# j-wilson/GPflowPILCO

Measured on AMD Instinct MI355X. Metric: moment_matched_rollout_step_elements_per_sec, higher is better.
Workload: dtype f32; 1 GPU; C3 (BASELINE configs[2]): N=2000 d=8 D=8 H=40 fp32 drift moment-match step / closed rollout; recipe=baseline: BASELINE.md recipe: lengthscales log-U[0.3,3], GP-prior targets, fresh mu~U[0,1]^d / Sigm~; N=2000, d=8, D=8, H=40, B_per_gpu=256, B_total=256, B_this_rank=256, parallelism=dp1 over B (weak), recipe=baseline, steps_requested=418, diag_pairs=f64, offdiag_pairs=f32

## Files before the change

### __graft_entry__.py

```python
import os
import subprocess
import sys

ROOT = os.path.dirname(os.path.abspath(__file__))
if ROOT not in sys.path:
  sys.path.insert(0, ROOT)


def build() -> None:
  script = os.path.join(ROOT, "gpflowpilco_amd", "csrc", "build.sh")
  subprocess.run(["bash", script], check=True)
  subprocess.run(["bash", os.path.join(ROOT, "tests", "hostcheck", "build.sh")], check=True)
  subprocess.run(["bash", os.path.join(ROOT, "tests", "hostcheck", "build_nd.sh")], check=True)
  subprocess.run(["bash", os.path.join(ROOT, "tests", "hostcheck", "build_mix.sh")], check=True)
  subprocess.run(["bash", os.path.join(ROOT, "tests", "hostcheck", "build_gram.sh")], check=True)
  subprocess.run(["bash", os.path.join(ROOT, "tests", "hostcheck", "build_predict.sh")], check=True)
  subprocess.run(["bash", os.path.join(ROOT, "tests", "hostcheck", "build_gram_stats.sh")], check=True)
  subprocess.run(["bash", os.path.join(ROOT, "tests", "hostcheck", "build_lanes.sh")], check=True)
  subprocess.run(["bash", os.path.join(ROOT, "tests", "devcheck", "build.sh")], check=True)
  import gpflowpilco_amd
  from gpflowpilco_amd import _lib
  lib = _lib.lib()
  assert lib.mm_abi_version() >= 1
  for name in _lib.SIGNATURES:
    getattr(lib, name)
  import gpflowpilco_amd.moment_matching
  import gpflowpilco_amd.dynamics


def smoke() -> None:
  import numpy as np
  import torch
  from gpflowpilco_amd import ops
  from gpflowpilco_amd.moment_matching import GaussianMoments, moment_matching
  from gpflowpilco_amd.synthetic import make_inputs, make_svgp
  from oracle import mm_oracle as mo

  assert torch.cuda.is_available(), "smoke() needs a GPU"
  dev = torch.device("cuda:0")
  L = d = 4
  syn = make_svgp(L, 96, d, seed=33)
  mu, Sigma = make_inputs(4, d, seed=5, scale=0.1, lo=0.3, hi=0.7)
  po = mo.SVGPParams(Z=np.broadcast_to(syn.Z, (L, 96, d)).copy(), lengthscales=syn.lengthscales,
                     variance=syn.variance, q_mu=syn.q_mu, q_sqrt=syn.q_sqrt, whiten=True)
  f1o, Sffo, cro = mo.mm_gauss_svgp_mo(mu, Sigma, po)
  muH, SH = mo.rollout_closed(mu, Sigma, po, 3)
  model = syn.to_model(dev)
  for dtype, tol in ((torch.float64, 1e-6), (torch.float32, 2e-4)):
    x = GaussianMoments((torch.tensor(mu, dtype=dtype, device=dev),
                         torch.tensor(Sigma, dtype=dtype, device=dev)), centered=True)
    m = moment_matching(x, model)
    for got, want in ((m.y.mean(), f1o), (m.y.covariance(), Sffo), (m.cross[0], cro)):
      err = np.abs(got.double().cpu().numpy() - want).max() / np.abs(want).max()
      assert err < tol, (dtype, err)
    pm = model.packed(dtype, True, dev)
    m1, S1 = ops.rollout_closed(pm, x.mean(), x.covariance(), 3)
    pm.check_status(4)
    assert np.abs(m1.double().cpu().numpy() - muH).max() / np.abs(muH).max() < tol
    assert np.abs(S1.double().cpu().numpy() - SH).max() / np.abs(SH).max() < tol
  from gpflowpilco_amd.synthetic import make_cartpole_like
  from oracle import mm_compose_oracle as co
  drift_s, pol_s = make_cartpole_like(M_drift=40, M_policy=12, seed=7, device=str(dev))
  drift, pol = drift_s.to_model(dev), pol_s.to_model(dev)
  H, active, scale, shift = 3, (1,), 2.0, -0.5
  mx, Sx = make_inputs(2, 4, seed=9, scale=0.05, lo=0.3, hi=0.7)
  target, precis = np.array([0.0, 1.0, 0.0, 0.0, 0.0]), 4.0 * np.eye(5)
  f64 = torch.float64
  roll = ops.ComposedRollout(drift.packed(f64, True, dev), pol.packed(f64, False, dev), nx=4, active_dims=active,
                             head_scale=scale, head_shift=shift, target=torch.tensor(target, dtype=f64, device=dev),
                             precis=torch.tensor(precis, dtype=f64, device=dev))
  m_H, S_H, cost = roll(torch.tensor(mx, dtype=f64, device=dev), torch.tensor(Sx, dtype=f64, device=dev), H)
  po_d = mo.SVGPParams(Z=np.broadcast_to(drift_s.Z, (4, 40, 6)).copy(), lengthscales=drift_s.lengthscales, variance=drift_s.variance,
                       q_mu=drift_s.q_mu, q_sqrt=drift_s.q_sqrt, whiten=True)
  po_p = mo.SVGPParams(Z=pol_s.Z[None].copy(), lengthscales=pol_s.lengthscales, variance=pol_s.variance, q_mu=pol_s.q_mu,
                       q_sqrt=pol_s.q_sqrt, whiten=True)
  loss_o, traj_o = co.policy_rollout_loss(mx, Sx, po_d, lambda st: co.mm_policy(st, po_p, scale, shift), active, target, precis, H, keep=True)
  assert np.abs(m_H.cpu().numpy() - traj_o[-1][0]).max() < 1e-8 and np.abs(S_H.cpu().numpy() - traj_o[-1][1]).max() < 1e-8
  assert abs(float(cost.sum()) - float(np.sum(loss_o))) < 1e-8
  from gpflowpilco_amd import bijectors as tfb, dynamics, models as gp
  from gpflowpilco_amd.components import GaussianObjective, TrigonometricEncoder
  from gpflowpilco_amd.loops import get_state_initializer, policy_loss_closure
  pol.q_mu.requires_grad_(True)
  policy = gp.InverseLinkWrapper(gp.KernelRegressor(pol), invlink=tfb.Chain([tfb.Scale(scale), tfb.Shift(shift), tfb.NormalCDF()]))
  system = dynamics.DynamicalSystem(drift=drift, policy=policy, encoder=TrigonometricEncoder(active_dims=active),
                                    solver=dynamics.MomentMatchingEuler())
  objective = GaussianObjective(target=torch.tensor(target, dtype=f64, device=dev), precis=torch.tensor(precis, dtype=f64, device=dev))
  closure = policy_loss_closure(system, objective, get_state_initializer(torch.tensor(mx, dtype=f64, device=dev),
                                                                        torch.tensor(Sx, dtype=f64, device=dev)), H)
  loss = closure().sum()
  assert abs(float(loss.detach()) - float(np.sum(loss_o))) < 1e-8
  loss.backward()
  g = pol.q_mu.grad.clone()
  direction = torch.randn(pol.q_mu.shape, dtype=f64, device=dev, generator=torch.Generator(device=dev).manual_seed(3))
  vals = []
  with torch.no_grad():
    for sgn in (1.0, -1.0):
      pol.q_mu.add_(sgn * 1e-5 * direction)
      vals.append(float(closure().sum()))
      pol.q_mu.sub_(sgn * 1e-5 * direction)
  fd = (vals[0] - vals[1]) / 2e-5
  an = float((g * direction).sum())
  assert abs(fd - an) < 1e-6 * max(1.0, abs(fd)), (fd, an)
  syn3 = make_svgp(3, 200, 8, seed=35, ls_bounds=(0.6, 2.5))
  model3 = syn3.to_model(dev)
  mu3, S3 = make_inputs(2, 8, seed=6, scale=0.1, lo=0.3, hi=0.7)
  mu3, S3 = torch.tensor(mu3, dtype=torch.float32, device=dev), torch.tensor(S3, dtype=torch.float32, device=dev)
  gg = torch.Generator(device="cpu").manual_seed(4)
  g1, g2, g3 = (torch.randn(s, generator=gg, dtype=f64).to(dev) for s in ((2, 3), (2, 3, 3), (2, 8, 3)))
  got = ops.moment_match_backward(model3.packed(torch.float32, True, dev), mu3, S3, g1, g2, g3)
  want = ops.moment_match_backward(model3.packed(f64, True, dev), mu3.double(), S3.double(), g1, g2, g3)
  for a_, b_ in zip(got, want):
    assert float((a_ - b_).abs().amax()) < 1e-4 * float(b_.abs().amax())
  pm3 = model3.packed(torch.float32, True, dev)
  f1s, Sffs, crs, sums, gen = ops.moment_match_with_sums(pm3, mu3, S3)
  gs = ops.moment_match_backward(pm3, mu3, S3, g1, g2, g3, forward_generation=gen, sums=sums)
  pm3.check_status(2)
  po3 = mo.SVGPParams(Z=np.broadcast_to(syn3.Z, (3, 200, 8)).copy(), lengthscales=syn3.lengthscales, variance=syn3.variance,
                      q_mu=syn3.q_mu, q_sqrt=syn3.q_sqrt, whiten=True)
  _, Sff3o, _ = mo.mm_gauss_svgp_mo(mu3.double().cpu().numpy(), S3.double().cpu().numpy(), po3)
  assert np.abs(Sffs.double().cpu().numpy() - Sff3o).max() < 2e-5 * np.abs(Sff3o).max()
  assert all(torch.equal(x_, y_) for x_, y_ in zip(gs, got))
  print("smoke ok")


if __name__ == "__main__":
  build()
  if len(sys.argv) > 1 and sys.argv[1] == "smoke":
    smoke()
```

### gpflowpilco_amd/_lib.py

```python
from __future__ import annotations

import ctypes as C
import os

_HERE = os.path.dirname(os.path.abspath(__file__))
LIB_PATH = os.environ.get("GPFLOWPILCO_MM_LIB") or os.path.join(_HERE, "libgpflowpilco_mm.so")

MM_F32, MM_F64 = 0, 1
MM_DMAX = 32
MM_M_ALIGN = 128
MM_FULL_OUTPUT_COV = 1
MM_MODEL_UNCERTAINTY = 2
MM_FORCE_GENERIC = 4
MM_STAGE_DIAG = 8
MM_STAGE_OFFDIAG = 16
MM_STAGE_FINALIZE = 32
MM_FORCE_WORST_TIER = 64
MM_WORKSPACE_CURRENT = 128
MM_FORCE_ROUTE = 256
MM_NO_ROUTE = 512
MM_SUMS_CURRENT = 1024
MM_ISTAGE_OLD_SKIP_BOUND = 1 << 26
MM_ISTAGE_NO_BOUND_SKIP = 1 << 27
MM_ISTAGE_OLD_WMOM = 1 << 28

ERRORS = {
    -1: "MM_E_ARG: NULL pointer or non-positive size",
    -2: "MM_E_DIM: input dimension d exceeds MM_DMAX=32 or unsupported shape",
    -3: "MM_E_DTYPE: dtype must be MM_F32 or MM_F64",
    -4: "MM_E_WORKSPACE: workspace/packed buffer too small",
    -5: "MM_E_NO_C: model_uncertainty requested but the model was packed without C",
    -6: "MM_E_STATE: Euler update / closed rollout needs d == L and a full output covariance",
}

SIGNATURES = {
    "mm_abi_version": (C.c_int, []),
    "mm_packed_model_bytes": (C.c_size_t, [C.c_int] * 5),
    "mm_pack_model": (C.c_int, [C.c_void_p, C.c_size_t, C.c_int, C.c_int, C.c_int, C.c_int]
                      + [C.c_void_p] * 6 + [C.c_void_p]),
    "mm_pack_perm": (C.c_int, [C.c_void_p, C.c_size_t, C.c_int, C.c_int, C.c_int, C.c_int, C.c_void_p, C.c_void_p]),
    "mm_workspace_bytes": (C.c_size_t, [C.c_int] * 6),
    "mm_moment_match": (C.c_int, [C.c_void_p, C.c_size_t, C.c_int, C.c_int, C.c_int, C.c_int, C.c_int,
                                  C.c_void_p, C.c_void_p, C.c_int, C.c_double,
                                  C.c_void_p, C.c_void_p, C.c_void_p,
                                  C.c_void_p, C.c_size_t, C.c_void_p, C.c_void_p]),
    "mm_q_forward": (C.c_int, [C.c_void_p, C.c_size_t, C.c_int, C.c_int, C.c_int, C.c_int, C.c_int,
                               C.c_void_p, C.c_void_p, C.c_int,
                               C.c_void_p, C.c_void_p, C.c_void_p,
                               C.c_void_p, C.c_size_t, C.c_void_p, C.c_void_p]),
    "mm_Q_reduce_forward": (C.c_int, [C.c_void_p, C.c_size_t, C.c_int, C.c_int, C.c_int, C.c_int, C.c_int,
                                      C.c_int, C.c_double, C.c_void_p,
                                      C.c_void_p, C.c_size_t, C.c_void_p]),
    "mm_euler_update": (C.c_int, [C.c_int, C.c_int, C.c_int, C.c_double] + [C.c_void_p] * 8),
    "mm_expected_cost": (C.c_int, [C.c_int, C.c_int, C.c_int] + [C.c_void_p] * 6),
    "mm_offdiag_stats": (C.c_int, [C.c_void_p, C.c_size_t, C.c_int, C.c_int, C.c_int, C.c_int, C.c_int, C.c_int,
                                   C.c_void_p, C.c_size_t, C.c_void_p, C.c_void_p]),
    "mm_offdiag_worklist_len": (C.c_int, [C.c_int] * 6 + [C.c_void_p, C.c_size_t, C.c_void_p, C.c_void_p]),
    "mm_offdiag_skip_bounds": (C.c_int, [C.c_void_p, C.c_size_t, C.c_int, C.c_int, C.c_int, C.c_int, C.c_int, C.c_int,
                                         C.c_void_p, C.c_size_t, C.c_void_p, C.c_void_p, C.c_void_p]),
    "mm_route_estimates": (C.c_int, [C.c_void_p, C.c_size_t, C.c_int, C.c_int, C.c_int, C.c_int, C.c_int, C.c_int,
                                     C.c_void_p, C.c_size_t, C.c_void_p, C.c_void_p]),
    "mm_compose_workspace_bytes": (C.c_size_t, [C.c_int] * 4),
    "mm_compose_nd_workspace_bytes": (C.c_size_t, [C.c_int] * 5),
    "mm_compose_tape_bytes": (C.c_size_t, [C.c_int] * 6),
    "mm_compose_backward_workspace_bytes": (C.c_size_t, [C.c_int] * 4),
    "mm_policy_grad_bytes": (C.c_size_t, [C.c_int] * 3),
    "mm_compose_tape_bytes_nd": (C.c_size_t, [C.c_int] * 7),
    "mm_compose_backward_workspace_bytes_nd": (C.c_size_t, [C.c_int] * 6),
    "mm_policy_grad_bytes_nd": (C.c_size_t, [C.c_int] * 4),
    "mm_compose_nd_mixed_workspace_bytes": (C.c_size_t, [C.c_int] * 6),
    "mm_compose_tape_bytes_nd_mixed": (C.c_size_t, [C.c_int] * 8),
    "mm_compose_backward_workspace_bytes_nd_mixed": (C.c_size_t, [C.c_int] * 7),
    "mm_bwd_f32_supported": (C.c_int, [C.c_int]),
    "mm_backward_pair_aggregates_bytes": (C.c_size_t, [C.c_int] * 5),
    "mm_backward_pair_aggregates": (C.c_int, [C.c_void_p, C.c_size_t, C.c_int, C.c_int, C.c_int, C.c_int, C.c_int,
                                              C.c_void_p, C.c_void_p, C.c_int, C.c_void_p, C.c_size_t, C.c_void_p, C.c_size_t,
                                              C.c_void_p, C.c_size_t, C.c_void_p, C.c_void_p]),
    "mm_moment_match_backward_bytes": (C.c_size_t, [C.c_int] * 5),
    "mm_moment_match_backward_bytes_dtype": (C.c_size_t, [C.c_int] * 6),
    "mm_moment_match_backward": (C.c_int, [C.c_void_p, C.c_size_t, C.c_int, C.c_int, C.c_int, C.c_int, C.c_int,
                                           C.c_void_p, C.c_void_p, C.c_int,
                                           C.c_void_p, C.c_void_p, C.c_void_p,
                                           C.c_void_p, C.c_void_p, C.c_int,
                                           C.c_void_p, C.c_size_t, C.c_void_p, C.c_size_t,
                                           C.c_void_p, C.c_void_p]),
    "mm_moment_match_with_sums": (C.c_int, [C.c_void_p, C.c_size_t, C.c_int, C.c_int, C.c_int, C.c_int, C.c_int,
                                            C.c_void_p, C.c_void_p, C.c_int, C.c_double,
                                            C.c_void_p, C.c_void_p, C.c_void_p,
                                            C.c_void_p, C.c_size_t, C.c_void_p, C.c_size_t,
                                            C.c_void_p, C.c_void_p]),
    "mm_backward_bytes": (C.c_size_t, [C.c_int] * 5),
    "mm_backward_sums": (C.c_int, [C.c_void_p, C.c_size_t, C.c_int, C.c_int, C.c_int, C.c_int, C.c_int,
                                   C.c_void_p, C.c_int, C.c_void_p, C.c_size_t, C.c_void_p, C.c_size_t, C.c_void_p]),
    "mm_pathwise_eval": (C.c_int, [C.c_int] * 6 + [C.c_void_p] * 12),
    "mm_pathwise_rollout": (C.c_int, [C.c_int] * 7 + [C.c_double] + [C.c_void_p] * 13),
    "mm_pathwise_eval_jac": (C.c_int, [C.c_int] * 6 + [C.c_void_p] * 13),
    "mm_pathwise_eval_bound": (C.c_int, [C.c_int] * 6 + [C.c_void_p] * 13),
    "mm_pathwise_tape_bytes": (C.c_size_t, [C.c_int] * 6),
    "mm_pathwise_policy_rollout": (C.c_int, [C.c_int] * 5 + [C.c_double, C.c_int, C.c_int] + [C.c_void_p] * 10
                                   + [C.c_void_p, C.c_size_t, C.c_int, C.c_double, C.c_double]
                                   + [C.c_void_p] * 4 + [C.c_void_p, C.c_size_t, C.c_int, C.c_void_p]),
    "mm_pathwise_backward_scratch_bytes": (C.c_size_t, [C.c_int] * 3),
    "mm_pathwise_policy_rollout_backward": (C.c_int, [C.c_int] * 3 + [C.c_double, C.c_int, C.c_int, C.c_void_p]
                                            + [C.c_void_p, C.c_size_t, C.c_int, C.c_double, C.c_double]
                                            + [C.c_void_p] * 2 + [C.c_void_p, C.c_size_t] + [C.c_void_p] * 3
                                            + [C.c_void_p, C.c_size_t, C.c_void_p]),
    "mm_pathwise_policy_rollout_backward_seeded": (C.c_int, [C.c_int] * 3 + [C.c_double, C.c_int, C.c_int, C.c_void_p]
                                                   + [C.c_void_p, C.c_size_t, C.c_int, C.c_double, C.c_double]
                                                   + [C.c_void_p] * 2 + [C.c_void_p, C.c_size_t] + [C.c_void_p] * 4
                                                   + [C.c_void_p, C.c_size_t, C.c_void_p]),
    "mm_pathwise_tape_bytes_nd": (C.c_size_t, [C.c_int] * 7),
    "mm_pathwise_policy_rollout_nd": (C.c_int, [C.c_int] * 5 + [C.c_double, C.c_int, C.c_int, C.c_void_p, C.c_int]
                                      + [C.c_void_p] * 9
                                      + [C.c_void_p, C.c_size_t, C.c_int, C.c_void_p, C.c_void_p]
                                      + [C.c_void_p] * 4 + [C.c_void_p, C.c_size_t, C.c_int, C.c_void_p]),
    "mm_pathwise_backward_scratch_bytes_nd": (C.c_size_t, [C.c_int] * 4),
    "mm_pathwise_policy_rollout_backward_nd": (C.c_int, [C.c_int] * 3 + [C.c_double, C.c_int, C.c_int, C.c_void_p, C.c_int]
                                               + [C.c_void_p, C.c_size_t, C.c_int, C.c_void_p, C.c_void_p]
                                               + [C.c_void_p] * 2 + [C.c_void_p, C.c_size_t] + [C.c_void_p] * 3
                                               + [C.c_void_p, C.c_size_t, C.c_void_p]),
    "mm_pathwise_policy_rollout_backward_nd_seeded": (C.c_int, [C.c_int] * 3 + [C.c_double, C.c_int, C.c_int, C.c_void_p, C.c_int]
                                                      + [C.c_void_p, C.c_size_t, C.c_int, C.c_void_p, C.c_void_p]
                                                      + [C.c_void_p] * 2 + [C.c_void_p, C.c_size_t] + [C.c_void_p] * 4
                                                      + [C.c_void_p, C.c_size_t, C.c_void_p]),
    "mm_pathwise_policy_rollout_wide": (C.c_int, [C.c_int] * 5 + [C.c_double, C.c_int, C.c_int, C.c_void_p, C.c_int]
                                        + [C.c_void_p] * 9
                                        + [C.c_void_p, C.c_size_t, C.c_int, C.c_void_p, C.c_void_p]
                                        + [C.c_void_p] * 4 + [C.c_void_p, C.c_size_t, C.c_int, C.c_void_p]),
    "mm_pathwise_backward_scratch_bytes_wide": (C.c_size_t, [C.c_int] * 4),
    "mm_pathwise_policy_rollout_backward_wide": (C.c_int, [C.c_int] * 3 + [C.c_double, C.c_int, C.c_int, C.c_void_p, C.c_int]
                                                 + [C.c_void_p, C.c_size_t, C.c_int, C.c_void_p, C.c_void_p]
                                                 + [C.c_void_p] * 2 + [C.c_void_p, C.c_size_t] + [C.c_void_p] * 3
                                                 + [C.c_void_p, C.c_size_t, C.c_void_p]),
    "mm_pathwise_policy_rollout_backward_wide_seeded": (C.c_int, [C.c_int] * 3 + [C.c_double, C.c_int, C.c_int, C.c_void_p, C.c_int]
                                                        + [C.c_void_p, C.c_size_t, C.c_int, C.c_void_p, C.c_void_p]
                                                        + [C.c_void_p] * 2 + [C.c_void_p, C.c_size_t] + [C.c_void_p] * 4
                                                        + [C.c_void_p, C.c_size_t, C.c_void_p]),
    "mm_pathwise_tape_bytes_mixed": (C.c_size_t, [C.c_int] * 8),
    "mm_pathwise_policy_rollout_mixed": (C.c_int, [C.c_int] * 5 + [C.c_double, C.c_int, C.c_int, C.c_void_p, C.c_int]
                                         + [C.c_void_p] * 9
                                         + [C.c_void_p, C.c_size_t, C.c_int, C.c_void_p, C.c_void_p]
                                         + [C.c_void_p] * 4 + [C.c_void_p, C.c_size_t, C.c_int, C.c_void_p]
                                         + [C.c_int, C.c_void_p, C.c_void_p]),
    "mm_pathwise_policy_rollout_backward_mixed": (C.c_int, [C.c_int] * 3 + [C.c_double, C.c_int, C.c_int, C.c_void_p, C.c_int]
                                                  + [C.c_void_p, C.c_size_t, C.c_int, C.c_void_p, C.c_void_p]
                                                  + [C.c_void_p] * 2 + [C.c_void_p, C.c_size_t] + [C.c_void_p] * 4
                                                  + [C.c_void_p, C.c_size_t, C.c_void_p] + [C.c_int, C.c_void_p]),
    "mm_pathwise_eval_kern": (C.c_int, [C.c_int] * 6 + [C.c_void_p] * 12 + [C.c_int]),
    "mm_pathwise_rollout_kern": (C.c_int, [C.c_int] * 7 + [C.c_double] + [C.c_void_p] * 13 + [C.c_int]),
    "mm_pathwise_eval_jac_kern": (C.c_int, [C.c_int] * 6 + [C.c_void_p] * 13 + [C.c_int]),
    "mm_pathwise_eval_bound_kern": (C.c_int, [C.c_int] * 6 + [C.c_void_p] * 13 + [C.c_int]),
    "mm_pathwise_policy_rollout_kern": (C.c_int, [C.c_int] * 5 + [C.c_double, C.c_int, C.c_int, C.c_void_p, C.c_int]
                                        + [C.c_void_p] * 9
                                        + [C.c_void_p, C.c_size_t, C.c_int, C.c_void_p, C.c_void_p]
                                        + [C.c_void_p] * 4 + [C.c_void_p, C.c_size_t, C.c_int, C.c_void_p]
                                        + [C.c_int, C.c_void_p, C.c_void_p, C.c_int]),
    "mm_pathwise_mean_eval": (C.c_int, [C.c_int] * 5 + [C.c_void_p] * 10 + [C.c_int]),
    "mm_pathwise_policy_rollout_mean": (C.c_int, [C.c_int] * 4 + [C.c_double, C.c_int, C.c_int, C.c_void_p, C.c_int]
                                        + [C.c_void_p] * 6
                                        + [C.c_void_p, C.c_size_t, C.c_int, C.c_void_p, C.c_void_p]
                                        + [C.c_void_p] * 4 + [C.c_void_p, C.c_size_t, C.c_int, C.c_void_p]
                                        + [C.c_int, C.c_void_p, C.c_void_p, C.c_int]),
    "mm_pathwise_basis": (C.c_int, [C.c_int] * 5 + [C.c_void_p] * 9),
    "mm_pathwise_pack_stream": (C.c_int, [C.c_int] * 5 + [C.c_void_p] * 4),
    "mm_gram_workspace_bytes": (C.c_size_t, [C.c_int] * 4),
    "mm_gram_se": (C.c_int, [C.c_int] * 4 + [C.c_void_p] * 6),
    "mm_gram_se_backward": (C.c_int, [C.c_int] * 4 + [C.c_void_p] * 9 + [C.c_size_t, C.c_void_p]),
    "mm_predict_workspace_bytes": (C.c_size_t, [C.c_int] * 4),
    "mm_predict_se": (C.c_int, [C.c_int] * 4 + [C.c_void_p] * 10 + [C.c_size_t, C.c_void_p]),
    "mm_gram_stats_workspace_bytes": (C.c_size_t, [C.c_int] * 5),
    "mm_gram_stats_se": (C.c_int, [C.c_int] * 5 + [C.c_void_p] * 8 + [C.c_size_t, C.c_void_p]),
    "mm_gram_stats_se_backward": (C.c_int, [C.c_int] * 5 + [C.c_void_p] * 11 + [C.c_size_t, C.c_void_p]),
    "mm_rollout_closed": (C.c_int, [C.c_void_p, C.c_size_t, C.c_int, C.c_int, C.c_int, C.c_int, C.c_int, C.c_int,
                                    C.c_double, C.c_int, C.c_double,
                                    C.c_void_p, C.c_void_p, C.c_void_p, C.c_void_p,
                                    C.c_void_p, C.c_size_t, C.c_void_p, C.c_void_p]),
}


def _composed_rollout_signatures():
  P, Z, I, D = C.c_void_p, C.c_size_t, C.c_int, C.c_double
  prefix = [P, Z, I, I, I,  P, Z, I, I,  I, I, I, D, I, I, C.POINTER(C.c_int32)]
  heads = {"": [D, D], "_nd": [I, C.POINTER(D), C.POINTER(D)]}
  buffers = lambda n: [P, Z] * n + [P, P]
  roles = {"": [P] * 5 + buffers(3),
           "_taped": [P] * 3 + buffers(3),
           "_backward": [P, Z, P] + [P] * 3 + buffers(2),
           "_backward_seeded": [P, Z, P, P, P] + [P] * 3 + buffers(2)}
  sigs = {}
  for role, args in roles.items():
    stem, seeded, _ = role.partition("_seeded")
    for nd, head in heads.items():
      sigs[f"mm_rollout_composed{stem}{nd}{seeded}"] = (I, prefix + head + [P, P] + args)
  for role, mixing in (("", [P, P]), ("_taped", [P, P]), ("_backward", [P])):
    args = roles["_backward_seeded" if role == "_backward" else role]
    sigs[f"mm_rollout_composed{role}_nd_mixed"] = (I, prefix + heads["_nd"] + [P, P] + args + mixing)
  return sigs


SIGNATURES.update(_composed_rollout_signatures())


def _compose_wide_signatures():
  nd, seeded = (SIGNATURES[f"mm_rollout_composed_backward_nd{s}"][1] for s in ("", "_seeded"))
  return {"mm_compose_wide_backward": (C.c_int, list(nd)),
          "mm_compose_wide_backward_seeded": (C.c_int, list(seeded)),
          "mm_compose_wide_backward_mixed": (C.c_int, list(nd) + [C.c_void_p]),
          "mm_compose_wide_backward_mixed_seeded": (C.c_int, list(seeded) + [C.c_void_p]),
          "mm_compose_backward_workspace_bytes_wide": (C.c_size_t, [C.c_int] * 6),
          "mm_compose_backward_workspace_bytes_wide_mixed": (C.c_size_t, [C.c_int] * 7),
          "mm_compose_wide_dense_path": (C.c_int, [C.c_int])}


SIGNATURES.update(_compose_wide_signatures())

_lib = None


class MomentMatchingLibraryError(RuntimeError):
  pass


def lib():
  global _lib
  if _lib is None:
    if not os.path.exists(LIB_PATH):
      raise MomentMatchingLibraryError(
          f"{LIB_PATH} is missing: the HIP extension is not built and there is no CPU "
          "fallback. Run gpflowpilco_amd/csrc/build.sh (needs hipcc).")
    handle = C.CDLL(LIB_PATH)
    for name, (res, args) in SIGNATURES.items():
      fn = getattr(handle, name)
      fn.restype = res
      fn.argtypes = args
    _lib = handle
  return _lib


def check(rc: int, what: str):
  if rc == 0:
    return
  if rc < 0:
    raise ValueError(f"{what}: {ERRORS.get(rc, rc)}")
  raise MomentMatchingLibraryError(f"{what}: HIP error {rc}")
```

### gpflowpilco_amd/csrc/mm_common.h

```cpp
#pragma once
#include <stddef.h>
#include <stdint.h>
#include "../../include/gpflowpilco_mm.h"

static inline size_t mm_align_up(size_t x, size_t a) { return (x + a - 1) / a * a; }
static inline int mm_round_up_int(int x, int a) { return (x + a - 1) / a * a; }
static inline size_t mm_elem_size(int dtype) { return dtype == MM_F64 ? 8 : 4; }

#define MM_ISTAGE_NO_ROUTE (1 << 20)
#define MM_ISTAGE_ROUTE (1 << 21)
#define MM_ISTAGE_NO_M56 (1 << 22)
#define MM_ISTAGE_OLD_OFFDIAG (1 << 23)
#define MM_ISTAGE_OLD_SPOLY56 (1 << 24)
#define MM_ISTAGE_OLD_DIAG_MAP (1 << 25)
#define MM_ISTAGE_OLD_SKIP_BOUND (1 << 26)
#define MM_ISTAGE_NO_BOUND_SKIP (1 << 27)
#define MM_ISTAGE_OLD_WMOM (1 << 28)

#define MM_PW_KERNELS 3

static inline int mm_num_pairs(int L, int flags) {
  return (flags & MM_FULL_OUTPUT_COV) ? L * (L + 1) / 2 : L;
}

static inline int mm_moment_deg(int d) { return d <= 8 ? 4 : 2; }
static inline long long mm_binom(int n, int k) {
  if (k < 0 || k > n) return 0;
  long long r = 1;
  for (int i = 1; i <= k; ++i) r = r * (n - k + i) / i;
  return r;
}
static inline int mm_mono_count(int n, int d) { return (int)mm_binom(d + n - 1, n); }
static inline int mm_mono_offset(int n, int d) { int o = 0; for (int m = 0; m < n; ++m) o += mm_mono_count(m, d); return o; }
static inline size_t mm_rank_table_entries(int d) {
  const int dk = d <= 8 ? 8 : 32, deg = mm_moment_deg(d);
  size_t n = 0, p = 1;
  for (int k = 1; k <= deg; ++k) { p *= dk; n += p; }
  return n;
}
static inline int mm_moment_cols(int d) { return mm_round_up_int(mm_mono_offset(mm_moment_deg(d) + 1, d), 16); }
static inline int mm_moment56_off5(int d) { return d <= 8 ? mm_round_up_int(mm_mono_count(4, d), 128) : 0; }
static inline int mm_moment56_off6(int d) { return d <= 8 ? mm_moment56_off5(d) + mm_round_up_int(mm_mono_count(5, d), 128) : 0; }
static inline int mm_moment56_cols(int d) { return d <= 8 ? mm_moment56_off6(d) + mm_round_up_int(mm_mono_count(6, d), 128) : 0; }
struct MMTab56 { int ins[6], last[6], n_i16, mult2, mult3, n_f32; size_t bytes; };
static inline MMTab56 mm_tab56(int d) {
  MMTab56 t;
  int o = 0;
  for (int m = 0; m < 6; ++m) { t.ins[m] = o; o += mm_mono_count(m, d) * 8; }
  for (int k = 0; k < 6; ++k) { t.last[k] = o; o += mm_mono_count(k, d); }
  t.n_i16 = mm_round_up_int(o, 8);
  t.mult2 = 0; t.mult3 = mm_mono_count(2, d); t.n_f32 = mm_mono_count(2, d) + mm_mono_count(3, d);
  t.bytes = (size_t)t.n_i16 * 2 + (size_t)t.n_f32 * 4;
  return t;
}

struct MMModelLayout {
  int Mp, Kz, nd8, KMp;
  size_t Z64;
  size_t Zt64;
  size_t zbar;
  size_t ls2;
  size_t var;
  size_t meanc;
  size_t beta64;
  size_t Zc64;
  size_t Zc;
  size_t Zs3;
  size_t Zm;
  size_t zmax2;
  size_t rtab;
  size_t Zq2;
  size_t Zm56;
  size_t tab56;
  size_t perm;
  size_t skey;
  size_t zt2;
  size_t zt2s;
  size_t Cm;
  size_t total;
};
#define MM_SORT_MIN_M 256

static inline MMModelLayout mm_model_layout(int L, int M, int d, int dtype, int with_C) {
  MMModelLayout o;
  const size_t es = mm_elem_size(dtype), A = 256;
  o.Mp = mm_round_up_int(M, MM_M_ALIGN);
  o.Kz = mm_round_up_int(d, 2);
  o.nd8 = (d + 7) / 8;
  o.KMp = mm_moment_cols(d);
  size_t off = 0;
  o.Z64 = off;    off = mm_align_up(off + (size_t)L * M * d * 8, A);
  o.Zt64 = off;   off = mm_align_up(off + (size_t)L * d * o.Mp * 8, A);
  o.zbar = off;   off = mm_align_up(off + (size_t)L * d * 8, A);
  o.ls2 = off;    off = mm_align_up(off + (size_t)L * d * 8, A);
  o.var = off;    off = mm_align_up(off + (size_t)L * 8, A);
  o.meanc = off;  off = mm_align_up(off + (size_t)L * 8, A);
  o.beta64 = off; off = mm_align_up(off + (size_t)L * M * 8, A);
  o.Zc64 = off;   off = mm_align_up(off + (size_t)L * o.Mp * o.Kz * 8, A);
  o.Zc = o.Zc64;
  if (dtype != MM_F64) { o.Zc = off; off = mm_align_up(off + (size_t)L * o.Mp * o.Kz * es, A); }
  o.Zs3 = off;
  if (dtype != MM_F64) off = mm_align_up(off + (size_t)L * o.Mp * 24 * o.nd8 * 2, A);
  o.Zm = off;
  if (dtype != MM_F64) off = mm_align_up(off + (size_t)L * o.Mp * o.KMp * 8, A);
  o.zmax2 = off;  off = mm_align_up(off + (size_t)L * 8, A);
  o.rtab = off;   off = mm_align_up(off + mm_rank_table_entries(d) * 2, A);
  o.Zq2 = off;
  if (dtype != MM_F64 && d <= 8) off = mm_align_up(off + (size_t)L * (o.Mp / 32) * 8192, A);
  o.Zm56 = off;
  if (dtype != MM_F64 && d <= 8) off = mm_align_up(off + (size_t)L * 2 * mm_moment56_cols(d) * o.Mp * 2, A);
  o.tab56 = off;
  if (dtype != MM_F64 && d <= 8) off = mm_align_up(off + mm_tab56(d).bytes, A);
  o.perm = off;   off = mm_align_up(off + (size_t)L * o.Mp * 4, A);
  o.skey = off;   off = mm_align_up(off + (size_t)L * o.Mp * 8, A);
  o.zt2 = off;    off = mm_align_up(off + (size_t)L * (o.Mp / 32) * 4, A);
  o.zt2s = off;   off = mm_align_up(off + (size_t)L * (o.Mp / 32) * 4, A);
  o.Cm = off;
  if (with_C) off = mm_align_up(off + (size_t)L * o.Mp * o.Mp * 8, A);
  o.total = off;
  return o;
}

#define MM_MOM_SPLIT 2
#ifndef MM_COLLAPSE_BOUND2
#define MM_COLLAPSE_BOUND2 0.25f
#endif
#define MM_C6_X5_2 (1.0f / 256.0f)
#define MM_C6_X4_2 (1.0f / 1600.0f)
#define MM_C6_MAX 0.25f
#define MM_C6_C0 1.666663289e-01f
#define MM_C6_C1 4.166659713e-02f
#define MM_C6_C2 8.350561373e-03f
#define MM_C6_C3 1.391559141e-03f
#define MM_C6_SYS2 6.33e-6f
#define MM_C6_POLY_F64(x_) (((x_) * (x_)) * (x_) * fma(fma(fma((double)MM_C6_C3, (x_), (double)MM_C6_C2), (x_), (double)MM_C6_C1), (x_), (double)MM_C6_C0))
#ifndef MM_TIER1_DIV
#define MM_TIER1_DIV 20
#endif
#if MM_TIER1_DIV == 16
#define MM_TIER1_MAX 0.0625f
#define MM_REM1_C0 1.666936278e-01f
#define MM_REM1_C1 4.167173430e-02f
#elif MM_TIER1_DIV == 20
#define MM_TIER1_MAX 0.05f
#define MM_REM1_C0 1.666839272e-01f
#define MM_REM1_C1 4.166988656e-02f
#elif MM_TIER1_DIV == 24
#define MM_TIER1_MAX 0.041666668f
#define MM_REM1_C0 1.666786522e-01f
#define MM_REM1_C1 4.166889191e-02f
#elif MM_TIER1_DIV == 32
#define MM_TIER1_MAX 0.03125f
#define MM_REM1_C0 1.666734070e-01f
#define MM_REM1_C1 4.166791216e-02f
#else
#error "MM_TIER1_DIV must be 16, 20, 24 or 32"
#endif
#define MM_INSIDE_BOUND2 (0.998f * MM_C6_MAX * MM_C6_MAX)
#ifndef MM_ROUTE_TOL
#define MM_ROUTE_TOL 3.0e-4
#endif
#define MM_ROUTE_CSPLIT 8
static inline int mm_route_ncc(int NS, int npanel) { int n = NS / npanel; return n < 1 ? 1 : (n > MM_ROUTE_CSPLIT ? MM_ROUTE_CSPLIT : n); }
#define MM_EXP_CAP_F64 700.0
#define MM_EXP_CAP_F32 80.0f
#define MM_GEN_ROWS 64
#define MM_GEN_COLS 256
#define MM_PANEL_ROWS 256
__host__ __device__ inline int mm_mfma_groups(int Mp) { return (Mp + MM_PANEL_ROWS - 1) / MM_PANEL_ROWS * (MM_PANEL_ROWS / 64); }
__host__ __device__ inline int mm_f32p_list_off(int L) { return 4 + 2 * L; }
#define MM_F64_TILE 64

struct MMWorkspaceLayout {
  int Mp, P, Po, NS;
  size_t pairmat;
  size_t latmat;
  size_t rho1;
  size_t w64;
  size_t q64;
  size_t w;
  size_t lq;
  size_t rowD;
  size_t colD;
  size_t qhR;
  size_t qhC;
  size_t rowO;
  size_t colO;
  size_t f1raw;
  size_t whR;
  size_t whC;
  size_t mom;
  size_t amax;
  size_t amaxc;
  size_t gflag;
  size_t gperm;
  size_t s12;
  size_t gmax2;
  size_t gmax2s;
  size_t partB;
  size_t partC;
  size_t mu64;
  size_t estO;
  size_t rlist;
  size_t rcount;
  size_t rflag;
  size_t wsp;
  size_t mom56;
  size_t estS;
  size_t ilist;
  size_t plist;
  size_t s56;
  size_t f1s;
  size_t Sffs;
  size_t crs;
  size_t total;
};

static inline MMWorkspaceLayout mm_workspace_layout(int B, int L, int M, int d, int dtype, int flags) {
  MMWorkspaceLayout o;
  const size_t es = mm_elem_size(dtype), A = 256;
  o.Mp = mm_round_up_int(M, MM_M_ALIGN);
  o.P = mm_num_pairs(L, flags);
  o.Po = o.P - L;
  const int nrb = (o.Mp + MM_GEN_ROWS - 1) / MM_GEN_ROWS;
  const int ncb = (o.Mp + MM_GEN_COLS - 1) / MM_GEN_COLS;
  const int nt = o.Mp / MM_F64_TILE;
  int ns = nrb * ncb;
  if (nt * (nt + 1) / 2 > ns) ns = nt * (nt + 1) / 2;
  if (dtype == MM_F64 && o.Po > 0 && nt * nt > ns) ns = nt * nt;
  o.NS = ns;
  size_t off = 0;
  o.pairmat = off; off = mm_align_up(off + (size_t)B * o.P * (d * d + 1) * 8, A);
  o.latmat = off;  off = mm_align_up(off + (size_t)B * L * (2 * d * d + 2) * 8, A);
  o.rho1 = off;    off = mm_align_up(off + (size_t)B * L * o.Mp * 8, A);
  o.w64 = off;     off = mm_align_up(off + (size_t)B * L * o.Mp * 8, A);
  o.q64 = off;     off = mm_align_up(off + (size_t)B * L * o.Mp * 8, A);
  o.w = o.w64;
  o.lq = off;      off = mm_align_up(off + (size_t)B * L * o.Mp * 8, A);
  o.rowD = off;    off = mm_align_up(off + (size_t)B * L * o.Mp * 8, A);
  o.colD = off;    off = mm_align_up(off + (size_t)B * L * (d + 1) * o.Mp * 8, A);
  o.qhR = off;     off = mm_align_up(off + (size_t)B * L * o.Mp * 8, A);
  o.qhC = off;     off = mm_align_up(off + (size_t)B * L * o.Mp * 8, A);
  const size_t nrow = dtype == MM_F64 ? 1 : (size_t)(d + 1), ncol = dtype == MM_F64 ? (size_t)(d + 1) : 1;
  o.rowO = off;    off = mm_align_up(off + (size_t)B * o.Po * nrow * o.Mp * es, A);
  o.colO = off;    off = mm_align_up(off + (size_t)B * o.Po * ncol * o.Mp * es, A);
  o.f1raw = off;   off = mm_align_up(off + (size_t)B * L * 8, A);
  const size_t nwh = dtype == MM_F64 ? 0 : (size_t)B * o.Po * o.Mp;
  o.whR = off;     off = mm_align_up(off + nwh * 8, A);
  o.whC = off;     off = mm_align_up(off + nwh * 8, A);
  o.mom = off;     off = mm_align_up(off + (dtype == MM_F64 ? 0 : (size_t)B * o.Po * 2 * MM_MOM_SPLIT * mm_moment_cols(d) * 8), A);
  o.amax = off;    off = off + (size_t)B * o.Po * 4;
  o.amaxc = off;   off = mm_align_up(off + (size_t)B * o.Po * 4, A);
  o.gflag = off;   off = mm_align_up(off + (dtype == MM_F64 ? 0 : (size_t)B * o.Po * (o.Mp / 64)), A);
  o.gmax2 = off;   off = mm_align_up(off + (dtype == MM_F64 ? 0 : (size_t)B * o.Po * (o.Mp / 64) * 4), A);
  o.gmax2s = off;  off = mm_align_up(off + (dtype == MM_F64 ? 0 : (size_t)B * o.Po * (o.Mp / 64) * 4), A);
  o.gperm = off;   off = mm_align_up(off + (dtype == MM_F64 || L < 2 ? 0 : ((size_t)L * (L - 1) * B + 3 * L) * 4), A);
  o.s12 = off;     off = mm_align_up(off + (size_t)B * o.Po * 8, A);
  o.partB = off;   off = mm_align_up(off + (size_t)B * o.P * o.NS * 8, A);
  o.partC = off;   off = mm_align_up(off + (size_t)B * L * o.NS * 8, A);
  const size_t nro = dtype == MM_F64 ? 0 : (size_t)B * o.Po;
  o.mu64 = off;    off = mm_align_up(off + (size_t)B * d * 8, A);
  o.estO = off;    off = mm_align_up(off + nro * ((o.Mp + MM_PANEL_ROWS - 1) / MM_PANEL_ROWS) * 4, A);
  o.rlist = off;   off = mm_align_up(off + nro * 4, A);
  o.rcount = off;  off = mm_align_up(off + 16, A);
  o.rflag = off;   off = mm_align_up(off + nro * 4, A);
  const size_t n56 = (dtype == MM_F64 || d > 8) ? 0 : (size_t)B * o.Po;
  o.wsp = off;     off = mm_align_up(off + n56 * 4 * o.Mp * 2, A);
  o.mom56 = off;   off = mm_align_up(off + n56 * 2 * mm_moment56_cols(d) * 4, A);
  o.estS = off;    off = mm_align_up(off + n56 * 4, A);
  o.s56 = off;     off = mm_align_up(off + n56 * 8, A);
  o.ilist = off;   off = mm_align_up(off + n56 * 4 + 16, A);
  o.plist = off;   off = mm_align_up(off + (n56 ? (n56 + mm_f32p_list_off(L)) * 4 : 0), A);
  o.f1s = off;     off = mm_align_up(off + (size_t)B * L * es, A);
  o.Sffs = off;    off = mm_align_up(off + (size_t)B * L * L * es, A);
  o.crs = off;     off = mm_align_up(off + (size_t)B * d * L * es, A);
  o.total = off;
  return o;
}
```

### gpflowpilco_amd/csrc/mm_moments.hip

```cpp
#include <hip/hip_runtime.h>
#include <math.h>
#include "mm_common.h"
#include "mm_mono.h"

typedef double f64x4m __attribute__((ext_vector_type(4)));
typedef double f64x2m __attribute__((ext_vector_type(2)));

#define MM_GEMM_RB 64
#define MM_GEMM_NB 128
#define MM_GEMM_KB 32
#define MM_GEMM_AS 34
#define MM_GEMM_BS 144

__device__ __forceinline__ void mm_decode_pair_m(int p, int L, int& a, int& a2) {
  int r = p - L, i = 0;
  while (r >= L - 1 - i) { r -= L - 1 - i; ++i; }
  a = i; a2 = i + 1 + r;
}

__global__ __launch_bounds__(256) __attribute__((amdgpu_waves_per_eu(2, 2))) void k_wmom_gemm(const double* __restrict__ whR, const double* __restrict__ whC,
                                                      const double* __restrict__ Zm, int KMp, int L, int Mp, int B, int Po,
                                                      int nrb, int ncb, int nwork, int col_deg3,
                                                      const unsigned int* __restrict__ amaxc, const double* __restrict__ zmax2,
                                                      const int* __restrict__ gperm, double* __restrict__ mom) {
  const int orig = blockIdx.x;
  const int xcd = orig & 7, slot = orig >> 3;
  const int qn = nwork >> 3, rn = nwork & 7;
  int wi = (xcd < rn ? xcd * (qn + 1) : rn * (qn + 1) + (xcd - rn) * qn) + slot;
  const int rb = wi % nrb; wi /= nrb;
  const int ks = wi % MM_MOM_SPLIT; wi /= MM_MOM_SPLIT;
  const int cb = wi % ncb; wi /= ncb;
  const int a = wi;
  const int R = (L - 1) * B;
  auto row_item = [&](int r, int& b, int& po, int& side, int& acol) {
    const int which = r / B;
    b = r - which * B;
    const int ap = which < a ? which : which + 1;
    const int lo = ap < a ? ap : a, hi = ap < a ? a : ap;
    po = lo * (L - 1) - lo * (lo - 1) / 2 + (hi - lo - 1);
    side = ap < a ? 1 : 0;
    acol = hi;
  };
  const double* tab = Zm + (size_t)a * Mp * KMp;
  const int tid = threadIdx.x, wv = tid >> 6, lane = tid & 63, l15 = lane & 15, kq = lane >> 4;
  const int* perm = nullptr;
  if (cb * MM_GEMM_NB >= col_deg3) {
    if (gperm != nullptr) {
      if (rb * MM_GEMM_RB >= gperm[(size_t)L * R + a]) return;
      perm = gperm + (size_t)a * R;
    } else {
      const int r = rb * MM_GEMM_RB + lane;
      bool c = false;
      if (amaxc != nullptr && r < R) {
        int b, po, side, acol;
        row_item(r, b, po, side, acol);
        c = mm_item_collapsed(amaxc[(size_t)b * Po + po]);
      }
      if (!__any(c)) return;
    }
  }
  const int kslice = Mp / MM_MOM_SPLIT;
  const int k_begin = ks * kslice, nkb = kslice / MM_GEMM_KB;

  __shared__ double As[MM_GEMM_RB * MM_GEMM_AS];
  __shared__ double Bs[MM_GEMM_KB * MM_GEMM_BS];

  const int ar = tid >> 2, ak = (tid & 3) * 8;
  int arow = rb * MM_GEMM_RB + ar;
  arow = arow < R ? arow : R - 1;
  int ab, apo, aside, aacol;
  row_item(perm ? perm[arow] : arow, ab, apo, aside, aacol);
  const double* aptr = (aside ? whC : whR) + ((size_t)ab * Po + apo) * Mp + k_begin + ak;

  const int bk = tid >> 3, bc = (tid & 7) * 16;
  const int col0 = cb * MM_GEMM_NB + bc;
  const bool bvalid = col0 < KMp;
  const double* bptr = tab + (size_t)(k_begin + bk) * KMp + (bvalid ? col0 : 0);
  double2 ra[4], rbv[8];
  auto load_regs = [&](int kb) {
    const double* ap = aptr + kb * MM_GEMM_KB;
#pragma unroll
    for (int i = 0; i < 4; ++i) ra[i] = *reinterpret_cast<const double2*>(ap + 2 * i);
    const double* bp = bptr + (size_t)kb * MM_GEMM_KB * KMp;
#pragma unroll
    for (int i = 0; i < 8; ++i) rbv[i] = *reinterpret_cast<const double2*>(bp + 2 * i);
  };
  f64x4m acc[4][2];
#pragma unroll
  for (int rt = 0; rt < 4; ++rt)
#pragma unroll
    for (int ct = 0; ct < 2; ++ct) acc[rt][ct] = (f64x4m){0.0, 0.0, 0.0, 0.0};

  load_regs(0);
  for (int kb = 0; kb < nkb; ++kb) {
    __syncthreads();
#pragma unroll
    for (int i = 0; i < 4; ++i) *reinterpret_cast<double2*>(&As[ar * MM_GEMM_AS + ak + 2 * i]) = ra[i];
#pragma unroll
    for (int i = 0; i < 8; ++i)
      *reinterpret_cast<double2*>(&Bs[bk * MM_GEMM_BS + bc + 2 * ((i + (tid & 7)) & 7)]) = bvalid ? rbv[i] : make_double2(0.0, 0.0);
    __syncthreads();
    load_regs(kb + 1 < nkb ? kb + 1 : kb);
#pragma unroll
    for (int s = 0; s < MM_GEMM_KB / 4; ++s) {
      double av[4], bv[2];
#pragma unroll
      for (int rt = 0; rt < 4; ++rt) av[rt] = As[(rt * 16 + l15) * MM_GEMM_AS + 4 * s + kq];
#pragma unroll
      for (int ct = 0; ct < 2; ++ct)
        bv[ct] = Bs[(4 * s + kq) * MM_GEMM_BS + wv * 32 + ct * 16 + 2 * (((l15 >> 1) + 2 * wv + ct) & 7) + (l15 & 1)];
#pragma unroll
      for (int rt = 0; rt < 4; ++rt)
#pragma unroll
        for (int ct = 0; ct < 2; ++ct)
          acc[rt][ct] = __builtin_amdgcn_mfma_f64_16x16x4f64(av[rt], bv[ct], acc[rt][ct], 0, 0, 0);
    }
  }
#pragma unroll
  for (int rt = 0; rt < 4; ++rt)
#pragma unroll
    for (int r = 0; r < 4; ++r) {
      const int row = rb * MM_GEMM_RB + rt * 16 + kq + 4 * r;
      if (row >= R) continue;
      int b, po, side, acol;
      row_item(perm ? perm[row] : row, b, po, side, acol);
      double* o = mom + ((((size_t)b * Po + po) * 2 + side) * MM_MOM_SPLIT + ks) * KMp;
#pragma unroll
      for (int ct = 0; ct < 2; ++ct) {
        const int col = cb * MM_GEMM_NB + wv * 32 + ct * 16 + l15;
        if (col < KMp) o[col] = acc[rt][ct][r];
      }
    }
}

#define MM_GEMM1_MAXT 11
#define MM_GEMM1_BS(NT_) ((NT_) * 16 + (((NT_) & 1) ? 0 : 16))
#define MM_GEMM1_LDS(NT_) ((size_t)(MM_GEMM_RB * MM_GEMM_AS + MM_GEMM_KB * MM_GEMM1_BS(NT_)) * sizeof(double))

template <int NT, class OutRow>
__device__ __forceinline__ void mm_wmom_rows(const double* __restrict__ aptr, const double* __restrict__ bptr, int KMp, int nkb,
                                             double* __restrict__ As, double* __restrict__ Bs, int tid, OutRow&& out_row) {
  constexpr int BS = MM_GEMM1_BS(NT), W2 = NT * 8;
  const int wv = tid >> 6, lane = tid & 63, l15 = lane & 15, kq = lane >> 4;
  const int ar = tid >> 2, ak = (tid & 3) * 8;
  int bsrc[NT], bdst[NT];
#pragma unroll
  for (int i = 0; i < NT; ++i) {
    const int c = tid + 256 * i, row = c / W2, cp = c - row * W2;
    bsrc[i] = row * KMp + 2 * cp;
    bdst[i] = row * BS + 2 * cp;
  }
  f64x2m ra[4], rbv[NT];
  f64x4m acc[NT];
#define MM_G1_LOAD(kb_)                                                                                             \
  do {                                                                                                              \
    const double* ap_ = aptr + (kb_) * MM_GEMM_KB;                                                                  \
    _Pragma("unroll") for (int i = 0; i < 4; ++i) ra[i] = *reinterpret_cast<const f64x2m*>(ap_ + 2 * i);           \
    const double* bp_ = bptr + (size_t)(kb_) * MM_GEMM_KB * KMp;                                                    \
    _Pragma("unroll") for (int i = 0; i < NT; ++i) rbv[i] = *reinterpret_cast<const f64x2m*>(bp_ + bsrc[i]);       \
  } while (0)
#pragma unroll
  for (int ct = 0; ct < NT; ++ct) acc[ct] = (f64x4m){0.0, 0.0, 0.0, 0.0};
  MM_G1_LOAD(0);
  for (int kb = 0; kb < nkb; ++kb) {
    __syncthreads();
#pragma unroll
    for (int i = 0; i < 4; ++i) *reinterpret_cast<f64x2m*>(&As[ar * MM_GEMM_AS + ak + 2 * i]) = ra[i];
#pragma unroll
    for (int i = 0; i < NT; ++i) *reinterpret_cast<f64x2m*>(&Bs[bdst[i]]) = rbv[i];
    __syncthreads();
    MM_G1_LOAD(kb + 1 < nkb ? kb + 1 : kb);
#pragma unroll
    for (int s = 0; s < MM_GEMM_KB / 4; ++s) {
      const double av = As[(wv * 16 + l15) * MM_GEMM_AS + 4 * s + kq];
      double bv[NT];
#pragma unroll
      for (int ct = 0; ct < NT; ++ct) bv[ct] = Bs[(4 * s + kq) * BS + ct * 16 + l15];
#pragma unroll
      for (int ct = 0; ct < NT; ++ct) acc[ct] = __builtin_amdgcn_mfma_f64_16x16x4f64(av, bv[ct], acc[ct], 0, 0, 0);
    }
  }
#pragma unroll
  for (int r = 0; r < 4; ++r) {
    double* o = out_row(r);
    if (o == nullptr) continue;
#pragma unroll
    for (int ct = 0; ct < NT; ++ct) o[ct * 16] = acc[ct][r];
  }
#undef MM_G1_LOAD
}

template <int NT_HI, int NT_LO>
__global__ __launch_bounds__(256) __attribute__((amdgpu_waves_per_eu(2, 2))) void k_wmom_gemm1(
    const double* __restrict__ whR, const double* __restrict__ whC, const double* __restrict__ Zm, int KMp, int L, int Mp, int B,
    int Po, int nrb, int nwork, int col0, const int* __restrict__ gperm, double* __restrict__ mom) {
  static_assert(NT_LO <= NT_HI && NT_HI <= MM_GEMM1_MAXT, "column tiles per workgroup");
  const int orig = blockIdx.x;
  const int xcd = orig & 7, slot = orig >> 3;
  const int qn = nwork >> 3, rn = nwork & 7;
  int wi = (xcd < rn ? xcd * (qn + 1) : rn * (qn + 1) + (xcd - rn) * qn) + slot;
  const int ks = wi % MM_MOM_SPLIT; wi /= MM_MOM_SPLIT;
  const int rb = wi % nrb; wi /= nrb;
  const int a = wi;
  const int R = (L - 1) * B;
  auto row_item = [&](int r, int& b, int& po, int& side) {
    const int which = r / B;
    b = r - which * B;
    const int ap = which < a ? which : which + 1;
    const int lo = ap < a ? ap : a, hi = ap < a ? a : ap;
    po = lo * (L - 1) - lo * (lo - 1) / 2 + (hi - lo - 1);
    side = ap < a ? 1 : 0;
  };
  const int* perm = gperm != nullptr ? gperm + (size_t)a * R : nullptr;
  const bool all_tiles = NT_LO == NT_HI || rb * MM_GEMM_RB < gperm[(size_t)L * R + a];
  const int tid = threadIdx.x, wv = tid >> 6, lane = tid & 63, l15 = lane & 15, kq = lane >> 4;
  const int kslice = Mp / MM_MOM_SPLIT;
  const int k_begin = ks * kslice, nkb = kslice / MM_GEMM_KB;

  extern __shared__ double sm_g1[];
  double* As = sm_g1;
  double* Bs = sm_g1 + MM_GEMM_RB * MM_GEMM_AS;

  int arow = rb * MM_GEMM_RB + (tid >> 2);
  arow = arow < R ? arow : R - 1;
  int ab, apo, aside;
  row_item(perm ? perm[arow] : arow, ab, apo, aside);
  const double* aptr = (aside ? whC : whR) + ((size_t)ab * Po + apo) * Mp + k_begin + (tid & 3) * 8;
  const double* bptr = Zm + ((size_t)a * Mp + k_begin) * KMp + col0;

  auto out_row = [&](int r) -> double* {
    const int row = rb * MM_GEMM_RB + wv * 16 + kq + 4 * r;
    if (row >= R) return nullptr;
    int b, po, side;
    row_item(perm ? perm[row] : row, b, po, side);
    return mom + ((((size_t)b * Po + po) * 2 + side) * MM_MOM_SPLIT + ks) * KMp + col0 + l15;
  };
  if (all_tiles) mm_wmom_rows<NT_HI>(aptr, bptr, KMp, nkb, As, Bs, tid, out_row);
  else mm_wmom_rows<NT_LO>(aptr, bptr, KMp, nkb, As, Bs, tid, out_row);
}

__global__ __launch_bounds__(1024) void k_wmom_perm(const unsigned int* __restrict__ amaxc, const double* __restrict__ zmax2, int L, int B,
                                                    int Po, int* __restrict__ gperm) {
  const int a = blockIdx.x, tid = threadIdx.x, wv = tid >> 6, lane = tid & 63;
  const int R = (L - 1) * B;
  __shared__ int wsum[3][16];
  __shared__ int tot[3];
  int* out = gperm + (size_t)a * R;
  int cnt[3] = {0, 0, 0};
  auto cls_of = [&](int r) {
    const int which = r / B, b = r - which * B;
    const int ap = which < a ? which : which + 1;
    const int lo = ap < a ? ap : a, hi = ap < a ? a : ap;
    const int po = lo * (L - 1) - lo * (lo - 1) / 2 + (hi - lo - 1);
    const unsigned int ac = amaxc[(size_t)b * Po + po];
    const float x2 = mm_collapse_bound2(ac, zmax2[hi]);
    return !mm_item_collapsed(ac) ? 3 : (x2 > MM_C6_X5_2 ? 0 : (x2 > MM_C6_X4_2 ? 1 : 2));
  };
  for (int r = tid; r < R; r += 1024) { const int c = cls_of(r); if (c < 3) ++cnt[c]; }
#pragma unroll
  for (int c = 0; c < 3; ++c) {
#pragma unroll
    for (int off = 32; off > 0; off >>= 1) cnt[c] += __shfl_down(cnt[c], off, 64);
    if (lane == 0) wsum[c][wv] = cnt[c];
  }
  __syncthreads();
  if (tid < 3) { int t = 0; for (int w = 0; w < 16; ++w) t += wsum[tid][w]; tot[tid] = t; }
  __syncthreads();
  int ofs[3] = {0, tot[0], tot[0] + tot[1]};
  int ofs_n = 0;
  for (int r0 = 0; r0 < R; r0 += 1024) {
    const int r = r0 + tid;
    const bool in = r < R;
    const int c = in ? cls_of(r) : 4;
    int before[3], ctot[3];
    __syncthreads();
#pragma unroll
    for (int k = 0; k < 3; ++k) {
      const unsigned long long bal = __ballot(c == k);
      before[k] = __popcll(bal & ((1ull << lane) - 1ull));
      if (lane == 0) wsum[k][wv] = __popcll(bal);
    }
    __syncthreads();
    int nfront_before = 0, nfront_tot = 0;
#pragma unroll
    for (int k = 0; k < 3; ++k) {
      int wb = 0, ct = 0;
#pragma unroll
      for (int w = 0; w < 16; ++w) { if (w < wv) wb += wsum[k][w]; ct += wsum[k][w]; }
      before[k] += wb; ctot[k] = ct;
      nfront_before += before[k]; nfront_tot += ct;
    }
    if (in) {
      if (c < 3) out[ofs[c] + before[c]] = r;
      else out[R - 1 - (ofs_n + (tid - nfront_before))] = r;
    }
    const int nin = R - r0 < 1024 ? R - r0 : 1024;
#pragma unroll
    for (int k = 0; k < 3; ++k) ofs[k] += ctot[k];
    ofs_n += nin - nfront_tot;
  }
  if (tid == 0) {
    gperm[(size_t)L * R + a] = tot[0] + tot[1] + tot[2];
    gperm[(size_t)L * R + L + a] = tot[0] + tot[1];
    gperm[(size_t)L * R + 2 * L + a] = tot[0];
  }
}

__device__ __forceinline__ double mm_block_sum256m(double v, double* red) {
#pragma unroll
  for (int off = 32; off > 0; off >>= 1) v += __shfl_down(v, off, 64);
  __syncthreads();
  if ((threadIdx.x & 63) == 0) red[threadIdx.x >> 6] = v;
  __syncthreads();
  return red[0] + red[1] + red[2] + red[3];
}

template <int DK, int LB>
__global__ __launch_bounds__(256) void k_spoly(const double* __restrict__ mom, int KMp, const double* __restrict__ pairmat,
                                               const double* __restrict__ zbar, const double* __restrict__ zmax2,
                                               const unsigned int* __restrict__ amax, const unsigned int* __restrict__ amaxc,
                                               const float* __restrict__ mu,
                                               int L, int d, int P, int deg, int allow_collapse,
                                               int off1, int off2, int off3, int off4, const short* __restrict__ rtab,
                                               double c0, double c1, double* __restrict__ s12) {
  extern __shared__ double sm[];
  const int po = blockIdx.x, b = blockIdx.y, tid = threadIdx.x;
  const int Po = P - L, p = L + po;
  int a, a2;
  mm_decode_pair_m(p, L, a, a2);
  const int dn = 1 << (LB * deg);
#define MM_PADI(i_) ((i_) + ((i_) >> 5))
  double* T = sm;
  double* U = T + MM_PADI(dn);
  double* nh = U + MM_PADI(dn >> LB);
  double* qh = nh + KMp;
  double* Gs = qh + KMp;
  double* dmu = Gs + DK * DK;
  __shared__ double red[4];
  {
    const double* nm = mom + (((size_t)b * Po + po) * 2 + 0) * MM_MOM_SPLIT * KMp;
    const double* qm = mom + (((size_t)b * Po + po) * 2 + 1) * MM_MOM_SPLIT * KMp;
    for (int k = tid; k < KMp; k += 256) {
      double sn = 0.0, sq = 0.0;
#pragma unroll
      for (int t = 0; t < MM_MOM_SPLIT; ++t) { sn += nm[t * KMp + k]; sq += qm[t * KMp + k]; }
      nh[k] = sn; qh[k] = sq;
    }
    const double* pm = pairmat + ((size_t)b * P + p) * (d * d + 1);
    for (int idx = tid; idx < DK * DK; idx += 256) {
      const int i = idx >> LB, j = idx & (DK - 1);
      Gs[idx] = (i < d && j < d) ? pm[i * d + j] : 0.0;
    }
    const bool rcen = mm_rows_recentred(amax[(size_t)b * Po + po]);
    if (tid < DK) dmu[tid] = (tid < d && !rcen) ? (double)mu[(size_t)b * d + tid] - zbar[a * d + tid] : 0.0;
  }
  __syncthreads();
  const bool coll = allow_collapse && deg >= 3 && mm_item_collapsed(amaxc[(size_t)b * Po + po]);
  const int nmax = coll ? deg : 2;
  double Gr[DK == 8 ? 64 : 1];
  if constexpr (DK == 8) {
#pragma unroll
    for (int i = 0; i < 64; ++i) Gr[i] = Gs[i];
  }
  double total = 0.0;
  for (int n = nmax; n >= 1; --n) {
    const double an = n == 1 ? 1.0 : n == 2 ? 0.5 : n == 3 ? c0 : c1;
    const int dsz = 1 << (LB * n);
    const int offn = n == 1 ? off1 : n == 2 ? off2 : n == 3 ? off3 : off4;
    const short* rtn = rtab + (((1 << (LB * n)) - DK) / (DK - 1));
    for (int idx = tid; idx < dsz; idx += 256) {
      const int r = rtn[idx];
      T[MM_PADI(idx)] = r >= 0 ? qh[offn + r] : 0.0;
    }
    __syncthreads();
    for (int t = 0; t < n; ++t) {
      const int sh = LB * t, nfib = dsz >> LB;
      for (int f = tid; f < nfib; f += 256) {
        const int lo = f & ((1 << sh) - 1), hi = f >> sh;
        const int base = (hi << (sh + LB)) + lo;
        double v[DK];
#pragma unroll
        for (int l = 0; l < DK; ++l) v[l] = T[MM_PADI(base + (l << sh))];
        if constexpr (DK == 8) {
#pragma unroll
          for (int k = 0; k < 8; ++k) {
            double s = 0.0;
#pragma unroll
            for (int l = 0; l < 8; ++l) s = fma(Gr[k * 8 + l], v[l], s);
            T[MM_PADI(base + (k << sh))] = s;
          }
        } else {
#pragma unroll 2
          for (int k = 0; k < DK; ++k) {
            double s = 0.0;
#pragma unroll
            for (int l = 0; l < DK; ++l) s = fma(Gs[k * DK + l], v[l], s);
            T[MM_PADI(base + (k << sh))] = s;
          }
        }
      }
      __syncthreads();
    }
    double* cur = T;
    double* oth = U;
    int ksz = dsz;
    double sign_binom = 1.0;
    for (int k = n; k >= 0; --k) {
      const int offk = k == 0 ? 0 : k == 1 ? off1 : k == 2 ? off2 : k == 3 ? off3 : off4;
      double part = 0.0;
      const short* rtk = rtab + (k ? (((1 << (LB * k)) - DK) / (DK - 1)) : 0);
      for (int idx = tid; idx < ksz; idx += 256) {
        const int r = k ? rtk[idx] : 0;
        if (r >= 0) part = fma(cur[MM_PADI(idx)], nh[offk + r], part);
      }
      total = fma(an * sign_binom, part, total);
      if (k == 0) break;
      const int nsz = ksz >> LB;
      for (int idx = tid; idx < nsz; idx += 256) {
        double s = 0.0;
#pragma unroll
        for (int l = 0; l < DK; ++l) s = fma(cur[MM_PADI(l * nsz + idx)], dmu[l], s);
        oth[MM_PADI(idx)] = s;
      }
      __syncthreads();
      double* tsw = cur; cur = oth; oth = tsw;
      ksz = nsz;
      sign_binom = -sign_binom * (double)k / (double)(n - k + 1);
    }
    __syncthreads();
  }
  const double tot = mm_block_sum256m(total, red);
  if (tid == 0) s12[(size_t)b * Po + po] = tot + nh[0] * qh[0];
#undef MM_PADI
}

#define MM_SPW_WAVES 4
__device__ __forceinline__ void mm_wave_sync_m() {
  __builtin_amdgcn_fence(__ATOMIC_RELEASE, "wavefront");
  __builtin_amdgcn_wave_barrier();
  __builtin_amdgcn_fence(__ATOMIC_ACQUIRE, "wavefront");
}
static inline int mm_spw_slice(int ncs) { return 512 + 16 + 64 + 2 + 2 * ncs + 64 + 8; }

__global__ __launch_bounds__(64 * MM_SPW_WAVES) void k_spoly_wave8(const double* __restrict__ mom, int KMp, const double* __restrict__ pairmat,
                                                                   const double* __restrict__ zbar, const unsigned int* __restrict__ amax,
                                                                   const unsigned int* __restrict__ amaxc, const float* __restrict__ mu,
                                                                   int L, int d, int P, int B, int allow_collapse,
                                                                   int off1, int off2, int off3, int off4, int ncs, int slice,
                                                                   const short* __restrict__ rtab, double c0,
                                                                   double* __restrict__ s12) {
  constexpr int DK = 8, LB = 3, DEG = 3;
  extern __shared__ double sm[];
  const int lane = threadIdx.x & 63, wv = threadIdx.x >> 6;
  const int Po = P - L;
  const int item = blockIdx.x * MM_SPW_WAVES + wv;
  if (item >= B * Po) return;
  const int b = item / Po, po = item - b * Po, p = L + po;
  int a, a2;
  mm_decode_pair_m(p, L, a, a2);
  constexpr int dn = 1 << (LB * DEG);
#define MM_PADI(i_) ((i_) + ((i_) >> 5))
  double* T = sm + (size_t)wv * slice;
  double* U = T + MM_PADI(dn);
  double* nh = U + MM_PADI(dn >> LB);
  double* qh = nh + ncs;
  double* Gs = qh + ncs;
  double* dmu = Gs + DK * DK;
  const bool coll = allow_collapse && mm_item_collapsed(amaxc[(size_t)b * Po + po]);
  const int nmax = coll ? DEG : 2;
  {
    const int ncol = coll ? off4 : off3;
    const double* nm = mom + (((size_t)b * Po + po) * 2 + 0) * MM_MOM_SPLIT * KMp;
    const double* qm = mom + (((size_t)b * Po + po) * 2 + 1) * MM_MOM_SPLIT * KMp;
    for (int k = lane; k < ncol; k += 64) {
      double sn = 0.0, sq = 0.0;
#pragma unroll
      for (int t = 0; t < MM_MOM_SPLIT; ++t) { sn += nm[t * KMp + k]; sq += qm[t * KMp + k]; }
      nh[k] = sn; qh[k] = sq;
    }
    const double* pm = pairmat + ((size_t)b * P + p) * (d * d + 1);
    {
      const int i = lane >> LB, j = lane & (DK - 1);
      Gs[lane] = (i < d && j < d) ? pm[i * d + j] : 0.0;
    }
    const bool rcen = mm_rows_recentred(amax[(size_t)b * Po + po]);
    if (lane < DK) dmu[lane] = (lane < d && !rcen) ? (double)mu[(size_t)b * d + lane] - zbar[a * d + lane] : 0.0;
  }
  mm_wave_sync_m();
  double Gr[64];
#pragma unroll
  for (int i = 0; i < 64; ++i) Gr[i] = Gs[i];
  double total[4] = {0.0, 0.0, 0.0, 0.0};
  for (int n = nmax; n >= 1; --n) {
    const double an = n == 1 ? 1.0 : n == 2 ? 0.5 : c0;
    const int dsz = 1 << (LB * n);
    const int offn = n == 1 ? off1 : n == 2 ? off2 : off3;
    const short* rtn = rtab + (((1 << (LB * n)) - DK) / (DK - 1));
    for (int idx = lane; idx < dsz; idx += 64) {
      const int r = rtn[idx];
      T[MM_PADI(idx)] = r >= 0 ? qh[offn + r] : 0.0;
    }
    mm_wave_sync_m();
    for (int t = 0; t < n; ++t) {
      const int sh = LB * t, nfib = dsz >> LB;
      for (int f = lane; f < nfib; f += 64) {
        const int lo = f & ((1 << sh) - 1), hi = f >> sh;
        const int base = (hi << (sh + LB)) + lo;
        double v[DK];
#pragma unroll
        for (int l = 0; l < DK; ++l) v[l] = T[MM_PADI(base + (l << sh))];
#pragma unroll
        for (int k = 0; k < 8; ++k) {
          double s = 0.0;
#pragma unroll
          for (int l = 0; l < 8; ++l) s = fma(Gr[k * 8 + l], v[l], s);
          T[MM_PADI(base + (k << sh))] = s;
        }
      }
      mm_wave_sync_m();
    }
    double* cur = T;
    double* oth = U;
    int ksz = dsz;
    double sign_binom = 1.0;
    for (int k = n; k >= 0; --k) {
      const int offk = k == 0 ? 0 : k == 1 ? off1 : k == 2 ? off2 : off3;
      const short* rtk = rtab + (k ? (((1 << (LB * k)) - DK) / (DK - 1)) : 0);
#pragma unroll
      for (int v = 0; v < 4; ++v) {
        double part = 0.0;
        for (int idx = lane + 64 * v; idx < ksz; idx += 256) {
          const int r = k ? rtk[idx] : 0;
          if (r >= 0) part = fma(cur[MM_PADI(idx)], nh[offk + r], part);
        }
        total[v] = fma(an * sign_binom, part, total[v]);
      }
      if (k == 0) break;
      const int nsz = ksz >> LB;
      for (int idx = lane; idx < nsz; idx += 64) {
        double s = 0.0;
#pragma unroll
        for (int l = 0; l < DK; ++l) s = fma(cur[MM_PADI(l * nsz + idx)], dmu[l], s);
        oth[MM_PADI(idx)] = s;
      }
      mm_wave_sync_m();
      double* tsw = cur; cur = oth; oth = tsw;
      ksz = nsz;
      sign_binom = -sign_binom * (double)k / (double)(n - k + 1);
    }
    mm_wave_sync_m();
  }
#pragma unroll
  for (int v = 0; v < 4; ++v) {
#pragma unroll
    for (int off = 32; off > 0; off >>= 1) total[v] += __shfl_down(total[v], off, 64);
  }
  if (lane == 0) {
    const double tot = total[0] + total[1] + total[2] + total[3];
    s12[(size_t)b * Po + po] = tot + nh[0] * qh[0];
  }
#undef MM_PADI
}

int mm_launch_wmom_full(const char* packed, const MMModelLayout& ml, char* ws, const MMWorkspaceLayout& wl,
                        int B, int L, int d, hipStream_t stream) {
  const int nrb = ((L - 1) * B + MM_GEMM_RB - 1) / MM_GEMM_RB, ncb = (ml.KMp + MM_GEMM_NB - 1) / MM_GEMM_NB;
  const long long nwork_ll = (long long)L * ncb * MM_MOM_SPLIT * nrb;
  if (nwork_ll <= 0 || nwork_ll > 0x7fffffffLL) return MM_E_DIM;
  hipLaunchKernelGGL(k_wmom_gemm, dim3((int)nwork_ll), dim3(256), 0, stream, (const double*)(ws + wl.whR),
                     (const double*)(ws + wl.whC), (const double*)(packed + ml.Zm), ml.KMp, L, wl.Mp, B, wl.Po, nrb, ncb,
                     (int)nwork_ll, 0x7fffffff , (const unsigned int*)nullptr, (const double*)(packed + ml.zmax2),
                     (const int*)nullptr, (double*)(ws + wl.mom));
  hipError_t e = hipGetLastError();
  return e == hipSuccess ? 0 : (int)e;
}

typedef void (*mm_gemm1_fn)(const double*, const double*, const double*, int, int, int, int, int, int, int, int, const int*, double*);
static mm_gemm1_fn mm_gemm1_kernel(int hi, int lo) {
#define MM_G1(HI_, LO_) if (hi == HI_ && lo == LO_) return k_wmom_gemm1<HI_, LO_>
  MM_G1(1, 1); MM_G1(2, 2); MM_G1(3, 3); MM_G1(4, 4); MM_G1(5, 5); MM_G1(6, 6); MM_G1(7, 7); MM_G1(8, 8); MM_G1(9, 9);
  MM_G1(10, 10); MM_G1(11, 11);
  MM_G1(2, 1); MM_G1(3, 1); MM_G1(4, 2); MM_G1(6, 2); MM_G1(8, 3); MM_G1(11, 3);
#undef MM_G1
  return nullptr;
}

static int mm_launch_wmom_onepass(const char* packed, const MMModelLayout& ml, char* ws, const MMWorkspaceLayout& wl, int B, int L,
                                  int ncol, int col_deg3, const int* gperm, hipStream_t stream) {
  const int nrb = ((L - 1) * B + MM_GEMM_RB - 1) / MM_GEMM_RB;
  const long long nwork_ll = (long long)L * MM_MOM_SPLIT * nrb;
  if (nwork_ll <= 0 || nwork_ll > 0x7fffffffLL) return MM_E_DIM;
  const int nt = (ncol + 15) / 16;
  const int npass = gperm != nullptr ? 1 : (nt + MM_GEMM1_MAXT - 1) / MM_GEMM1_MAXT;
  const int per = (nt + npass - 1) / npass;
  for (int p = 0; p < npass; ++p) {
    const int hi = nt - p * per < per ? nt - p * per : per;
    const int lo = gperm != nullptr ? (col_deg3 + 15) / 16 : hi;
    const mm_gemm1_fn fn = mm_gemm1_kernel(hi, lo < hi ? lo : hi);
    if (fn == nullptr || 16 * (p * per + hi) > ml.KMp) return MM_E_DIM;
    hipLaunchKernelGGL(fn, dim3((int)nwork_ll), dim3(256), MM_GEMM1_LDS(hi), stream, (const double*)(ws + wl.whR), (const double*)(ws + wl.whC),
                       (const double*)(packed + ml.Zm), ml.KMp, L, wl.Mp, B, wl.Po, nrb, (int)nwork_ll, 16 * p * per, gperm,
                       (double*)(ws + wl.mom));
    const hipError_t e = hipGetLastError();
    if (e != hipSuccess) return (int)e;
  }
  return 0;
}

int mm_launch_moments56(const char* packed, const MMModelLayout& ml, char* ws, const MMWorkspaceLayout& wl,
                        int B, int L, int d, int allow, int old_spoly56, hipStream_t stream);

int mm_launch_moments(const char* packed, const MMModelLayout& ml, char* ws, const MMWorkspaceLayout& wl,
                      int B, int L, int d, const void* mu_f32, int flags, hipStream_t stream) {
  const double* Zm = (const double*)(packed + ml.Zm);
  double* mom = (double*)(ws + wl.mom);
  const int deg = mm_moment_deg(d) >= 4 ? 3 : mm_moment_deg(d);
  const int ncol_fwd = mm_mono_offset(deg + 1, d);
  const int nrb = ((L - 1) * B + MM_GEMM_RB - 1) / MM_GEMM_RB, ncb = (ncol_fwd + MM_GEMM_NB - 1) / MM_GEMM_NB;
  const long long nwork_ll = (long long)L * ncb * MM_MOM_SPLIT * nrb;
  if (nwork_ll <= 0 || nwork_ll > 0x7fffffffLL) return MM_E_DIM;
  const int nwork = (int)nwork_ll;
  const int allow = (flags & (MM_FORCE_WORST_TIER | MM_ISTAGE_NO_M56)) ? 0 : 1;
  const int col_deg3 = mm_mono_offset(3, d);
  const bool some = allow && mm_moment_deg(d) >= 4;
  if (some) {
    hipLaunchKernelGGL(k_wmom_perm, dim3(L), dim3(1024), 0, stream, (const unsigned int*)(ws + wl.amaxc),
                       (const double*)(packed + ml.zmax2), L, B, wl.Po, (int*)(ws + wl.gperm));
    hipError_t ep = hipGetLastError();
    if (ep != hipSuccess) return (int)ep;
  }
  const bool old_wmom = (flags & MM_ISTAGE_OLD_WMOM) != 0;
  hipError_t e = hipSuccess;
  if (old_wmom) {
    hipLaunchKernelGGL(k_wmom_gemm, dim3(nwork), dim3(256), 0, stream, (const double*)(ws + wl.whR),
                       (const double*)(ws + wl.whC), Zm, ml.KMp, L, wl.Mp, B, wl.Po, nrb, ncb, nwork, col_deg3,
                       some ? (const unsigned int*)(ws + wl.amaxc) : (const unsigned int*)nullptr,
                       (const double*)(packed + ml.zmax2), some ? (const int*)(ws + wl.gperm) : (const int*)nullptr, mom);
    e = hipGetLastError();
    if (e != hipSuccess) return (int)e;
  } else {
    const int ncol = (mm_moment_deg(d) >= 4 && !some) ? col_deg3 : ncol_fwd;
    const int rc = mm_launch_wmom_onepass(packed, ml, ws, wl, B, L, ncol, col_deg3, some ? (const int*)(ws + wl.gperm) : (const int*)nullptr,
                                          stream);
    if (rc != 0) return rc;
  }
  const int off1 = mm_mono_offset(1, d), off2 = mm_mono_offset(2, d), off3 = mm_mono_offset(3, d), off4 = mm_mono_offset(4, d);
#define MM_SPOLY(DK_, LB_)                                                                                                       \
  do {                                                                                                                          \
    const int dn_ = 1 << (LB_ * deg);                                                                                           \
    const int up_ = dn_ >> LB_;                                                                                                 \
    const size_t shm_ = (size_t)(dn_ + (dn_ >> 5) + up_ + (up_ >> 5) + 2 * ml.KMp + DK_ * DK_ + DK_ + 8) * sizeof(double);      \
    hipLaunchKernelGGL((k_spoly<DK_, LB_>), dim3(wl.Po, B), dim3(256), shm_, stream, (const double*)mom, ml.KMp,                \
                       (const double*)(ws + wl.pairmat), (const double*)(packed + ml.zbar), (const double*)(packed + ml.zmax2), \
                       (const unsigned int*)(ws + wl.amax), (const unsigned int*)(ws + wl.amaxc), (const float*)mu_f32, L, d, wl.P, deg, allow, off1, off2, off3, off4, \
                       (const short*)(packed + ml.rtab),                                                                        \
                       (double)MM_C6_C0, (double)MM_C6_C1, (double*)(ws + wl.s12));                                             \
  } while (0)
  if (d <= 8 && !old_wmom) {
    const int ncs = (off4 + 7) & ~7;
    const int slice = mm_spw_slice(ncs);
    const int nitem = B * wl.Po;
    hipLaunchKernelGGL(k_spoly_wave8, dim3((nitem + MM_SPW_WAVES - 1) / MM_SPW_WAVES), dim3(64 * MM_SPW_WAVES),
                       (size_t)MM_SPW_WAVES * slice * sizeof(double), stream, (const double*)mom, ml.KMp,
                       (const double*)(ws + wl.pairmat), (const double*)(packed + ml.zbar), (const unsigned int*)(ws + wl.amax),
                       (const unsigned int*)(ws + wl.amaxc), (const float*)mu_f32, L, d, wl.P, B, allow, off1, off2, off3, off4,
                       ncs, slice, (const short*)(packed + ml.rtab), (double)MM_C6_C0, (double*)(ws + wl.s12));
  } else if (d <= 8) MM_SPOLY(8, 3); else MM_SPOLY(32, 5);
#undef MM_SPOLY
  e = hipGetLastError();
  if (e != hipSuccess) return (int)e;
  if (flags & MM_ISTAGE_NO_M56) {
    if (mm_moment56_cols(d) <= 0 || wl.Po <= 0) return 0;
    const hipError_t em = hipMemsetAsync(ws + wl.s56, 0xFF, (size_t)B * wl.Po * sizeof(double), stream);
    if (em != hipSuccess) return (int)em;
    const hipError_t es = hipMemsetAsync(ws + wl.estS, 0, (size_t)B * wl.Po * sizeof(float), stream);
    return es == hipSuccess ? 0 : (int)es;
  }
  return mm_launch_moments56(packed, ml, ws, wl, B, L, d, some ? 1 : 0, (flags & MM_ISTAGE_OLD_SPOLY56) ? 1 : 0, stream);
}

__global__ void k_offdiag_stats(const unsigned int* __restrict__ amax, const double* __restrict__ zmax2,
                                const unsigned char* __restrict__ gflag, int ng, int L, int Po, int n,
                                int32_t* __restrict__ out) {
  const int idx = blockIdx.x * blockDim.x + threadIdx.x;
  bool c = false, in = false, part = false;
  int groups = 0;
  if (idx < n) {
    int a, a2;
    mm_decode_pair_m(L + idx % Po, L, a, a2);
    const float b2 = mm_collapse_bound2(amax[idx], zmax2[a2]);
    c = b2 <= MM_COLLAPSE_BOUND2;
    in = b2 <= MM_INSIDE_BOUND2;
    part = !c && mm_item_collapsed(amax[n + idx]);
    for (int g = 0; g < ng; ++g) groups += gflag[(size_t)idx * ng + g] ? 1 : 0;
  }
  const unsigned long long m = __ballot(c), mi = __ballot(in), mp = __ballot(part);
  if ((threadIdx.x & 63) == 0 && m) atomicAdd(out, (int)__popcll(m));
  if ((threadIdx.x & 63) == 0 && mi) atomicAdd(out + 2, (int)__popcll(mi));
  if ((threadIdx.x & 63) == 0 && mp) atomicAdd(out + 4, (int)__popcll(mp));
#pragma unroll
  for (int off = 32; off > 0; off >>= 1) groups += __shfl_down(groups, off, 64);
  if ((threadIdx.x & 63) == 0 && groups) atomicAdd(out + 5, groups);
  if (idx == 0) out[1] = n;
}

extern "C" int mm_offdiag_stats(const void* packed, size_t packed_bytes, int L, int M, int d, int dtype, int B, int flags,
                                const void* workspace, size_t workspace_bytes, int32_t* out, void* stream) {
  if (!packed || !workspace || !out || L <= 0 || M <= 0 || d <= 0 || d > MM_DMAX || B <= 0) return MM_E_ARG;
  const MMModelLayout ml = mm_model_layout(L, M, d, dtype, 1);
  const MMWorkspaceLayout wl = mm_workspace_layout(B, L, M, d, dtype, flags);
  if (packed_bytes < ml.Cm || workspace_bytes < wl.total) return MM_E_WORKSPACE;
  hipStream_t s = (hipStream_t)stream;
  hipError_t e = hipMemsetAsync(out, 0, 6 * sizeof(int32_t), s);
  if (e != hipSuccess) return (int)e;
  if (dtype == MM_F32 && wl.Po > 0) {
    e = hipMemcpyAsync(out + 3, (const char*)workspace + wl.rcount + 4, sizeof(int32_t), hipMemcpyDeviceToDevice, s);
    if (e != hipSuccess) return (int)e;
  }
  if (dtype != MM_F32 || wl.Po == 0 || mm_moment_deg(d) < 4 || (flags & MM_FORCE_WORST_TIER)) return 0;
  const int n = B * wl.Po;
  hipLaunchKernelGGL(k_offdiag_stats, dim3((n + 255) / 256), dim3(256), 0, s, (const unsigned int*)((const char*)workspace + wl.amax),
                     (const double*)((const char*)packed + ml.zmax2), (const unsigned char*)((const char*)workspace + wl.gflag),
                     wl.Mp / MM_GROUP_ROWS, L, wl.Po, n, out);
  e = hipGetLastError();
  return e == hipSuccess ? 0 : (int)e;
}
```

### gpflowpilco_amd/csrc/mm_moments6.hip

```cpp
#include <hip/hip_runtime.h>
#include <math.h>
#include "mm_common.h"
#include "mm_mono.h"
#include "mm_f32_tile.h"
#include <atomic>
#include <type_traits>

__device__ __forceinline__ void mm6_decode_pair_o(int lp, int L, int& a, int& a2) {
  int r = lp, i = 0;
  while (r >= L - 1 - i) { r -= L - 1 - i; ++i; }
  a = i; a2 = i + 1 + r;
}

__global__ __launch_bounds__(256) void k_pack_zm56(char* packed, MMModelLayout lay, int L, int M, int d, int N56p,
                                                   const double* __restrict__ Z) {
  const int c = blockIdx.x, a = blockIdx.y, tid = threadIdx.x;
  const int n4 = mm_binom_i(d + 3, 4), n5 = mm_binom_i(d + 4, 5), n6 = mm_binom_i(d + 5, 6);
  const int off5 = ((n4 + 127) / 128) * 128;
  const int off6 = off5 + ((n5 + 127) / 128) * 128;
  const double* zbar = (const double*)(packed + lay.zbar) + (size_t)a * d;
  unsigned short* oh = (unsigned short*)(packed + lay.Zm56) + (((size_t)a * 2 + 0) * N56p + c) * lay.Mp;
  unsigned short* om = (unsigned short*)(packed + lay.Zm56) + (((size_t)a * 2 + 1) * N56p + c) * lay.Mp;
  int n = 0, k[6] = {0, 0, 0, 0, 0, 0};
  if (c < n4) { n = 4; mm_mono_unrank(c, 4, k); }
  else if (c >= off5 && c < off5 + n5) { n = 5; mm_mono_unrank(c - off5, 5, k); }
  else if (c >= off6 && c < off6 + n6) { n = 6; mm_mono_unrank(c - off6, 6, k); }
  for (int m = tid; m < lay.Mp; m += 256) {
    float vf = 0.0f;
    if (n && m < M) {
      double v = 1.0;
      for (int t = 0; t < n; ++t) v *= Z[((size_t)a * M + m) * d + k[t]] - zbar[k[t]];
      vf = (float)v;
    }
    const __bf16 h = (__bf16)vf;
    const __bf16 mid = (__bf16)(vf - (float)h);
    oh[m] = __builtin_bit_cast(unsigned short, h);
    om[m] = __builtin_bit_cast(unsigned short, mid);
  }
}

__global__ __launch_bounds__(256) void k_pack_tab56(char* packed, MMModelLayout lay, int d, MMTab56 t) {
  short* i16 = (short*)(packed + lay.tab56);
  float* f32 = (float*)(packed + lay.tab56 + (size_t)t.n_i16 * 2);
  const int tid = threadIdx.x;
  for (int m = 0; m < 6; ++m) {
    const int ns = mm_binom_i(d + m - 1, m);
    for (int idx = tid; idx < ns * 8; idx += 256) {
      const int J = idx >> 3, j = idx & 7;
      int k[6] = {0, 0, 0, 0, 0, 0}, kk[7];
      mm_mono_unrank(J, m, k);
      short r = 0;
      if (j < d) {
        int pos = 0;
        while (pos < m && k[pos] <= j) ++pos;
        for (int u = 0; u < pos; ++u) kk[u] = k[u];
        kk[pos] = j;
        for (int u = pos; u < m; ++u) kk[u + 1] = k[u];
        r = (short)mm_mono_rank(kk, m + 1);
      }
      i16[t.ins[m] + idx] = r;
    }
    for (int I = tid; I < ns; I += 256) {
      int k[6] = {0, 0, 0, 0, 0, 0};
      mm_mono_unrank(I, m, k);
      i16[t.last[m] + I] = (short)(m ? k[m - 1] : 0);
    }
  }
  for (int n = 2; n <= 3; ++n) {
    const int ns = mm_binom_i(d + n - 1, n);
    for (int I = tid; I < ns; I += 256) {
      int k[6] = {0, 0, 0, 0, 0, 0};
      mm_mono_unrank(I, n, k);
      double mult = 1.0;
      int run = 0;
      for (int u = 0; u < n; ++u) {
        mult *= (double)(u + 1);
        run = (u > 0 && k[u] == k[u - 1]) ? run + 1 : 1;
        mult /= (double)run;
      }
      f32[(n == 2 ? t.mult2 : t.mult3) + I] = (float)mult;
    }
  }
}

int mm_launch_pack56(char* packed, const MMModelLayout& lay, int L, int M, int d, const double* Z, hipStream_t s) {
  const int N56p = mm_moment56_cols(d);
  if (N56p <= 0) return 0;
  hipLaunchKernelGGL(k_pack_zm56, dim3(N56p, L), dim3(256), 0, s, packed, lay, L, M, d, N56p, Z);
  hipError_t e = hipGetLastError();
  if (e != hipSuccess) return (int)e;
  hipLaunchKernelGGL(k_pack_tab56, dim3(1), dim3(256), 0, s, packed, lay, d, mm_tab56(d));
  e = hipGetLastError();
  return e == hipSuccess ? 0 : (int)e;
}

#define MM6_TB 128
#define MM6_KB 32
#define MM6_STAGE_BYTES 32768

__global__ __launch_bounds__(256, 2) void k_wmom56_gemm(const unsigned short* __restrict__ wsp, const unsigned short* __restrict__ Zm56,
                                                        int N56p, int L, int Mp, int B, int Po, int nrb, int ncb, int nwork, int cb5, int cb6,
                                                        const int* __restrict__ gperm, float* __restrict__ mom56) {
  const int orig = blockIdx.x;
  const int xcd = orig & 7, slot = orig >> 3;
  const int qn = nwork >> 3, rn = nwork & 7;
  int wi = (xcd < rn ? xcd * (qn + 1) : rn * (qn + 1) + (xcd - rn) * qn) + slot;
  const int rb = wi % nrb; wi /= nrb;
  const int cb = wi % ncb; wi /= ncb;
  const int a = wi;
  const int R = (L - 1) * B;
  const int ncoll = gperm[(size_t)L * R + (cb < cb5 ? 0 : (cb < cb6 ? 1 : 2)) * L + a];
  if (rb * MM6_TB >= ncoll) return;
  const int* perm = gperm + (size_t)a * R;
  extern __shared__ __align__(1024) char lds[];
  int* orow = reinterpret_cast<int*>(lds + 2 * MM6_STAGE_BYTES);
  const int tid = threadIdx.x, wv = tid >> 6, lane = tid & 63, l31 = lane & 31, h = lane >> 5;
  auto row_item = [&](int r) {
    const int which = r / B, b = r - which * B;
    const int ap = which < a ? which : which + 1;
    const int lo = ap < a ? ap : a, hi = ap < a ? a : ap;
    const int po = lo * (L - 1) - lo * (lo - 1) / 2 + (hi - lo - 1);
    return ((b * Po + po) << 1) | (ap < a ? 1 : 0);
  };
  if (tid < MM6_TB) {
    const int r = rb * MM6_TB + tid;
    orow[tid] = r < ncoll ? row_item(perm[r]) : -1;
  }
  const bool isB = wv >= 2;
  const int part = wv & 1;
  unsigned int src_off[8];
#pragma unroll
  for (int i = 0; i < 8; ++i) {
    const int row = i * 16 + (lane >> 2);
    const int lc = (lane & 3) ^ ((row >> 2) & 3);
    if (isB) {
      src_off[i] = (unsigned int)((((size_t)a * 2 + part) * N56p + (size_t)cb * MM6_TB + row) * Mp) + lc * 8;
    } else {
      int r = rb * MM6_TB + row;
      r = r < ncoll ? r : ncoll - 1;
      src_off[i] = (unsigned int)(((size_t)row_item(perm[r]) * 2 + part) * Mp) + lc * 8;
    }
  }
  const unsigned short* src = isB ? Zm56 : wsp;
  auto stage = [&](int kb, int buf) {
    char* dst = lds + buf * MM6_STAGE_BYTES + (isB ? 16384 : 0) + part * 8192;
#pragma unroll
    for (int i = 0; i < 8; ++i)
      __builtin_amdgcn_global_load_lds((const __attribute__((address_space(1))) void*)(src + src_off[i] + kb * MM6_KB),
                                       (__attribute__((address_space(3))) void*)(dst + i * 1024), 16, 0, 0);
  };
  const int wr = wv >> 1, wc = wv & 1;
  f32x16 acc[2][2];
#pragma unroll
  for (int rt = 0; rt < 2; ++rt)
#pragma unroll
    for (int ct = 0; ct < 2; ++ct)
#pragma unroll
      for (int e = 0; e < 16; ++e) acc[rt][ct][e] = 0.0f;
  int fragA[2], fragB[2];
#pragma unroll
  for (int t = 0; t < 2; ++t) {
    fragA[t] = (wr * 64 + t * 32 + l31) * 64;
    fragB[t] = 16384 + (wc * 64 + t * 32 + l31) * 64;
  }
  const int swz = (l31 >> 2) & 3;
  const int nkb = Mp / MM6_KB;
  stage(0, 0);
  for (int kb = 0; kb < nkb; ++kb) {
    __syncthreads();
    if (kb + 1 < nkb) stage(kb + 1, (kb + 1) & 1);
    const char* base = lds + (kb & 1) * MM6_STAGE_BYTES;
#pragma unroll
    for (int ks = 0; ks < 2; ++ks) {
      const int ch = ((ks * 2 + h) ^ swz) * 16;
      bf16x8 Ah[2], Am[2], Th[2], Tm[2];
#pragma unroll
      for (int t = 0; t < 2; ++t) {
        Ah[t] = *reinterpret_cast<const bf16x8*>(base + fragA[t] + ch);
        Am[t] = *reinterpret_cast<const bf16x8*>(base + 8192 + fragA[t] + ch);
        Th[t] = *reinterpret_cast<const bf16x8*>(base + fragB[t] + ch);
        Tm[t] = *reinterpret_cast<const bf16x8*>(base + 8192 + fragB[t] + ch);
      }
#pragma unroll
      for (int rt = 0; rt < 2; ++rt)
#pragma unroll
        for (int ct = 0; ct < 2; ++ct) {
          acc[rt][ct] = __builtin_amdgcn_mfma_f32_32x32x16_bf16(Am[rt], Th[ct], acc[rt][ct], 0, 0, 0);
          acc[rt][ct] = __builtin_amdgcn_mfma_f32_32x32x16_bf16(Ah[rt], Tm[ct], acc[rt][ct], 0, 0, 0);
          acc[rt][ct] = __builtin_amdgcn_mfma_f32_32x32x16_bf16(Ah[rt], Th[ct], acc[rt][ct], 0, 0, 0);
        }
    }
  }
#pragma unroll
  for (int rt = 0; rt < 2; ++rt)
#pragma unroll
    for (int e = 0; e < 16; ++e) {
      const int item = orow[wr * 64 + rt * 32 + 8 * (e >> 2) + 4 * h + (e & 3)];
      if (item < 0) continue;
      float* o = mom56 + (size_t)item * N56p + (size_t)cb * MM6_TB + wc * 64 + l31;
#pragma unroll
      for (int ct = 0; ct < 2; ++ct) o[ct * 32] = acc[rt][ct][e];
    }
}

#ifndef MM6_THREADS
#define MM6_THREADS 768
#endif
#define MM6_WAVES (MM6_THREADS / 64)
#ifndef MM6_NC
#define MM6_NC 2
#endif
template <int K, bool TRANSG, int MODE, int NC = MM6_NC, int NW = MM6_WAVES>
__device__ __forceinline__ void mm6_step(const float* __restrict__ Tin, int nJin, int nI, float* __restrict__ Tout, int nJp,
                                         const short* __restrict__ ins, int d, const float (&G)[64], const float* __restrict__ multJ,
                                         int xs, float& acc, int wave, int lane) {
  const int chunks = (nJp + 64 * NC - 1) / (64 * NC);
  auto dots = [&](auto i0c, const float (&v)[NC][8], float (&s)[NC][8]) __attribute__((always_inline)) {
    constexpr int I0 = decltype(i0c)::value;
#pragma unroll
    for (int q = 0; q < NC; ++q)
#pragma unroll
      for (int i = I0; i < 8; ++i) s[q][i] = G[0 * 8 + i] * v[q][0];
#pragma unroll
    for (int j = 1; j < 8; ++j)
#pragma unroll
      for (int q = 0; q < NC; ++q)
#pragma unroll
        for (int i = I0; i < 8; ++i) s[q][i] = fmaf(G[j * 8 + i], v[q][j], s[q][i]);
  };
  auto body = [&](int I, int t, const int (&Jp)[NC], const bool (&jv)[NC], const int (&off)[NC][8], const float (&mj)[NC]) __attribute__((always_inline)) {
    const float* tin = Tin + I * nJin;
    float v[NC][8], s[NC][8];
#pragma unroll
    for (int q = 0; q < NC; ++q)
#pragma unroll
      for (int j = 0; j < 8; ++j) v[q][j] = tin[off[q][j]];
    if (t < 4) dots(std::integral_constant<int, 0>{}, v, s);
    else if (t < 6) dots(std::integral_constant<int, 4>{}, v, s);
    else dots(std::integral_constant<int, 6>{}, v, s);
#pragma unroll
    for (int i = 0; i < 8; ++i) {
      if (i >= t && i < d) {
        const int orow = I + mm_binom_i(i + K, K + 1);
        float m3 = 1.0f;
        if constexpr (MODE == 1 && K == 2) {
          const int a = I - ((t * (t + 1)) >> 1);
          m3 = a == t ? (i == t ? 1.0f : 3.0f) : (i == t ? 3.0f : 6.0f);
        } else if constexpr (MODE == 1 && K == 1) {
          m3 = i == t ? 1.0f : 2.0f;
        }
#pragma unroll
        for (int q = 0; q < NC; ++q) {
          if constexpr (MODE == 0) { if (jv[q]) Tout[orow * nJp + Jp[q]] = s[q][i]; }
          else if constexpr (MODE == 1) { if (jv[q]) Tout[orow * xs + Jp[q]] = (m3 * mj[q]) * s[q][i]; }
          else { if (jv[q]) acc = fmaf(s[q][i], Tout[Jp[q] * xs + orow], acc); }
        }
      }
    }
  };
  const int nunit = chunks * nI;
  const float rnI = 1.0f / (float)nI;
  int cprev = -1, off[NC][8], Jc[NC];
  bool jv[NC];
  float mj[NC];
#pragma unroll
  for (int q = 0; q < NC; ++q) { Jc[q] = 0; jv[q] = false; mj[q] = 0.0f; }
  for (int u = wave; u < nunit; u += NW) {
    int c = K == 0 ? u : (int)(((float)u + 0.5f) * rnI);
    c = __builtin_amdgcn_readfirstlane(c);
    const int I = K == 0 ? 0 : __builtin_amdgcn_readfirstlane(u - c * nI);
    if (c != cprev) {
      cprev = c;
#pragma unroll
      for (int q = 0; q < NC; ++q) {
        const int Jp = (c * NC + q) * 64 + lane;
        jv[q] = Jp < nJp;
        Jc[q] = jv[q] ? Jp : nJp - 1;
        const short4 ia = *reinterpret_cast<const short4*>(ins + (size_t)Jc[q] * 8);
        const short4 ib = *reinterpret_cast<const short4*>(ins + (size_t)Jc[q] * 8 + 4);
        off[q][0] = ia.x; off[q][1] = ia.y; off[q][2] = ia.z; off[q][3] = ia.w;
        off[q][4] = ib.x; off[q][5] = ib.y; off[q][6] = ib.z; off[q][7] = ib.w;
        if constexpr (MODE == 1) mj[q] = multJ[Jc[q]];
      }
    }
    int t = 0;
    if constexpr (K > 0) {
#pragma unroll
      for (int q = 1; q < 8; ++q) t += (I >= mm_binom_i(q + K - 1, K)) ? 1 : 0;
    }
    if (jv[0]) body(I, t, Jc, jv, off, mj);
  }
}

typedef float mm6_f2 __attribute__((ext_vector_type(2)));
typedef __attribute__((address_space(3))) float mm6_lds_f;
constexpr int mm6_cbinom(int n, int k) {
  if (k < 0 || k > n) return 0;
  int r = 1;
  for (int i = 1; i <= k; ++i) r = r * (n - k + i) / i;
  return r;
}
constexpr int mm6_sym8(int k) { return mm6_cbinom(8 + k - 1, k); }

template <int K, int MODE, int NJIN, int NJP, int XS, int NC, int NW>
__device__ __forceinline__ void mm6_step8(const float* __restrict__ Tin_, float* __restrict__ Tout_, const short* __restrict__ ins,
                                          const float (&G)[64], const float* __restrict__ multJ, float& acc, int wave, int lane) {
  asm volatile("" : "+v"(lane));
  unsigned a_in = (unsigned)(size_t)(const mm6_lds_f*)Tin_, a_out = (unsigned)(size_t)(mm6_lds_f*)Tout_;
  asm volatile("" : "+s"(a_in));
  asm volatile("" : "+s"(a_out));
  const mm6_lds_f* Tin = (const mm6_lds_f*)(size_t)a_in;
  mm6_lds_f* Tout = (mm6_lds_f*)(size_t)a_out;
  constexpr int NI = mm6_sym8(K);
  constexpr int CH = (NJP + 64 * NC - 1) / (64 * NC);
  constexpr int ST = MODE == 0 ? NJP : XS;
  static_assert(K >= 0 && K <= 2, "K of the n <= 6 chains");
  static_assert(mm6_cbinom(7 + K, K + 1) * ST * 4 < 65536, "the row term is a 16-bit ds offset");
  auto low = [](int t) constexpr { return mm6_cbinom(t + K - 1, K); };
  auto row = [](int i) constexpr { return mm6_cbinom(i + K, K + 1); };
  int off[NC][8], Jc[NC];
  bool jv[NC];
  float mj[NC];
  auto load_c = [&](int c) __attribute__((always_inline)) {
#pragma unroll
    for (int q = 0; q < NC; ++q) {
      const int Jp = (c * NC + q) * 64 + lane;
      jv[q] = Jp < NJP;
      Jc[q] = jv[q] ? Jp : NJP - 1;
      const short4 ia = *reinterpret_cast<const short4*>(ins + (size_t)Jc[q] * 8);
      const short4 ib = *reinterpret_cast<const short4*>(ins + (size_t)Jc[q] * 8 + 4);
      off[q][0] = ia.x; off[q][1] = ia.y; off[q][2] = ia.z; off[q][3] = ia.w;
      off[q][4] = ib.x; off[q][5] = ib.y; off[q][6] = ib.z; off[q][7] = ib.w;
      if constexpr (MODE == 1) mj[q] = multJ[Jc[q]];
    }
  };
  auto body = [&](auto i0c, int I, bool first) __attribute__((always_inline)) {
    constexpr int I0 = decltype(i0c)::value;
    const mm6_lds_f* tin = Tin + I * NJIN;
    float v[NC][8], s[NC][8];
#pragma unroll
    for (int q = 0; q < NC; ++q)
#pragma unroll
      for (int j = 0; j < 8; ++j) v[q][j] = tin[off[q][j]];
#pragma unroll
    for (int q = 0; q < NC; ++q) asm volatile("; unit %c1" : "+v"(v[q][0]) : "n"(I0 * 16 + K * 4 + MODE));
    mm6_f2 s2[NC][4];
#pragma unroll
    for (int q = 0; q < NC; ++q)
#pragma unroll
      for (int p = I0 / 2; p < 4; ++p) s2[q][p] = mm6_f2{G[2 * p], G[2 * p + 1]} * mm6_f2{v[q][0], v[q][0]};
#pragma unroll
    for (int j = 1; j < 8; ++j)
#pragma unroll
      for (int q = 0; q < NC; ++q)
#pragma unroll
        for (int p = I0 / 2; p < 4; ++p)
          s2[q][p] = __builtin_elementwise_fma(mm6_f2{G[j * 8 + 2 * p], G[j * 8 + 2 * p + 1]}, mm6_f2{v[q][j], v[q][j]}, s2[q][p]);
#pragma unroll
    for (int q = 0; q < NC; ++q)
#pragma unroll
      for (int p = I0 / 2; p < 4; ++p) {
        asm volatile("" : "+v"(s2[q][p]));
        s[q][2 * p] = s2[q][p].x; s[q][2 * p + 1] = s2[q][p].y;
      }
    if constexpr (MODE == 0) {
#pragma unroll
      for (int q = 0; q < NC; ++q) {
        mm6_lds_f* o = Tout + I * ST + Jc[q];
        if (jv[q]) {
          if (first) o[row(I0) * ST] = s[q][I0];
#pragma unroll
          for (int i = I0 + 1; i < 8; ++i) o[row(i) * ST] = s[q][i];
          asm volatile("; stores %c0" : : "n"((I0 * 16 + K * 4 + MODE) * 2 + q));
        }
      }
    } else if constexpr (MODE == 1) {
      float m_eq = 1.0f, m_gt = 2.0f;
      if constexpr (K == 2) {
        const bool aeq = first ? (I - low(I0) == I0) : (I - low(I0 + 1) == I0 + 1);
        m_eq = aeq ? 1.0f : 3.0f;
        m_gt = aeq ? 3.0f : 6.0f;
      }
      const float m_1 = first ? m_gt : m_eq;
#pragma unroll
      for (int q = 0; q < NC; ++q) {
        mm6_lds_f* o = Tout + I * ST + Jc[q];
        if (jv[q]) {
          if (first) o[row(I0) * ST] = (m_eq * mj[q]) * s[q][I0];
          o[row(I0 + 1) * ST] = (m_1 * mj[q]) * s[q][I0 + 1];
#pragma unroll
          for (int i = I0 + 2; i < 8; ++i) o[row(i) * ST] = (m_gt * mj[q]) * s[q][i];
          asm volatile("; stores %c0" : : "n"((I0 * 16 + K * 4 + MODE) * 2 + q));
        }
      }
    } else {
      const mm6_lds_f* x[NC];
#pragma unroll
      for (int q = 0; q < NC; ++q) x[q] = Tout + Jc[q] * ST + I;
      if (first) {
#pragma unroll
        for (int q = 0; q < NC; ++q) acc = (q == 0 || jv[q]) ? fmaf(s[q][I0], x[q][row(I0)], acc) : acc;
      }
#pragma unroll
      for (int i = I0 + 1; i < 8; ++i)
#pragma unroll
        for (int q = 0; q < NC; ++q) acc = (q == 0 || jv[q]) ? fmaf(s[q][i], x[q][row(i)], acc) : acc;
    }
    asm volatile("; end %c0" : : "n"(I0 * 16 + K * 4 + MODE));
  };
  auto unit = [&](int I) __attribute__((always_inline)) {
    if constexpr (K == 0) {
      body(std::integral_constant<int, 0>{}, 0, true);
    } else {
      if (I < low(4)) {
        if (I < low(2)) body(std::integral_constant<int, 0>{}, I, I < low(1));
        else body(std::integral_constant<int, 2>{}, I, I < low(3));
      } else {
        if (I < low(6)) body(std::integral_constant<int, 4>{}, I, I < low(5));
        else body(std::integral_constant<int, 6>{}, I, I < low(7));
      }
    }
  };
  if constexpr (CH == 1) {
    if (wave < NI) {
      load_c(0);
      for (int I = wave; I < NI; I += NW)
        if (jv[0]) unit(I);
    }
  } else if constexpr (NI == 1) {
    for (int c = wave; c < CH; c += NW) {
      load_c(c);
      if (jv[0]) unit(0);
    }
  } else if constexpr (MODE != 2 && NW % CH == 0) {
    const int c = wave % CH;
    load_c(c);
    for (int I = wave / CH; I < NI; I += NW / CH)
      if (jv[0]) unit(I);
  } else {
    int cprev = -1;
    for (int u = wave; u < CH * NI; u += NW) {
      const int c = u / NI, I = u - c * NI;
      if (c != cprev) { cprev = c; load_c(c); }
      if (jv[0]) unit(I);
    }
  }
}

template <bool D8, int K, bool TRANSG, int MODE, int NC, int NW, int KIN, int XS8>
__device__ __forceinline__ void mm6_do(const float* __restrict__ Tin, float* __restrict__ Tout, const int* sy, const short* __restrict__ tabi,
                                       const MMTab56& tb, int d, const float (&G)[64], const float* __restrict__ multJ, int xs,
                                       float& acc, int wave, int lane) {
  if constexpr (D8)
    mm6_step8<K, MODE, mm6_sym8(KIN), mm6_sym8(KIN - 1), XS8, NC, NW>(Tin, Tout, tabi + tb.ins[KIN - 1], G, multJ, acc, wave, lane);
  else
    mm6_step<K, TRANSG, MODE, NC, NW>(Tin, sy[KIN], sy[K], Tout, sy[KIN - 1], tabi + tb.ins[KIN - 1], d, G, multJ, xs, acc, wave, lane);
}

__global__ __launch_bounds__(256) void k_item_classes(const unsigned int* __restrict__ amaxc, const double* __restrict__ zmax2,
                                                      int L, int Po, int n, int allow, int* __restrict__ ilist,
                                                      double* __restrict__ s56, float* __restrict__ estS) {
  const int idx = blockIdx.x * 256 + threadIdx.x, lane = threadIdx.x & 63;
  int cls = 3;
  if (idx < n) {
    int a, a2;
    mm6_decode_pair_o(idx % Po, L, a, a2);
    const unsigned int ac = amaxc[idx];
    const float x2 = mm_collapse_bound2(ac, zmax2[a2]);
    cls = (!allow || !mm_item_collapsed(ac)) ? 3 : (x2 > MM_C6_X5_2 ? 0 : (x2 > MM_C6_X4_2 ? 1 : 2));
    if (cls == 3) { s56[idx] = 0.0; estS[idx] = 0.0f; }
  }
  const unsigned long long b01 = __ballot(cls == 0 || cls == 1), b2 = __ballot(cls == 2);
  int base01 = 0, base2 = 0;
  if (lane == 0) {
    if (b01) base01 = atomicAdd(ilist + 0, (int)__popcll(b01));
    if (b2) base2 = atomicAdd(ilist + 2, (int)__popcll(b2));
  }
  base01 = __shfl(base01, 0, 64); base2 = __shfl(base2, 0, 64);
  const unsigned long long below = (1ull << lane) - 1ull;
  if (cls == 0 || cls == 1) ilist[4 + base01 + __popcll(b01 & below)] = idx;
  if (cls == 2) ilist[4 + n - 1 - (base2 + __popcll(b2 & below))] = idx;
}

__device__ __forceinline__ float mm6_estS(float bound2, bool need5, bool need6, double r2, double c2) {
  const double X = sqrt((double)bound2), X3 = X * X * X;
  double amp = fmin(1.0, 64.0 * X3);
  if (!need6) amp += (double)MM_C6_C3 * X3 * X3 / 5.8e-10;
  if (!need5) amp += (double)MM_C6_C2 * X3 * X * X / 5.8e-10;
  return (float)fmin((double)MM_C6_SYS2 * (amp * amp) * r2 * c2, 3.0e38);
}

template <bool D8>
__global__ __launch_bounds__(MM6_THREADS) void k_spoly56(const float* __restrict__ mom56, int N56p, const double* __restrict__ pairmat,
                                                 const double* __restrict__ zmax2, const unsigned int* __restrict__ amaxc,
                                                 const unsigned char* __restrict__ gflag,
                                                 const double* __restrict__ whR, const double* __restrict__ whC,
                                                 const char* __restrict__ tab, MMTab56 tb, int L, int d_, int P, int Mp,
                                                 const int* __restrict__ ilist,
                                                 double* __restrict__ s56, float* __restrict__ estS) {
  extern __shared__ __align__(16) float sm6[];
  const int d = D8 ? 8 : d_;
  constexpr int NW = MM6_WAVES, NC = MM6_NC;
  const int tid = threadIdx.x;
  const int wave = __builtin_amdgcn_readfirstlane(tid >> 6), lane = tid & 63;
  const int Po = P - L;
  const int nitems = __builtin_amdgcn_readfirstlane(ilist[0]);
  for (int li = blockIdx.x; li < nitems; li += gridDim.x) {
  const size_t item = (size_t)__builtin_amdgcn_readfirstlane(ilist[4 + li]);
  const int b = (int)(item / Po), po = (int)(item - (size_t)b * Po);
  int a, a2;
  mm6_decode_pair_o(po, L, a, a2);
  const float bound2 = mm_collapse_bound2(amaxc[item], zmax2[a2]);
  int sy[7];
#pragma unroll
  for (int k = 0; k < 7; ++k) sy[k] = mm_binom_i(d + k - 1, k);
  const int n56 = sy[4] + sy[5] + sy[6];
  const int off5 = ((sy[4] + 127) / 128) * 128;
  const int off6 = off5 + ((sy[5] + 127) / 128) * 128;
  const bool need5 = bound2 > MM_C6_X4_2, need6 = bound2 > MM_C6_X5_2;
  const int xs = sy[3] + 1;
  float* nq = sm6;
  float* X = nq + 2 * n56;
  float* A = X + sy[3] * xs;
  float* Bf = A + sy[2] * sy[4];
  float* red = sm6 + ((2 * n56 + sy[3] * xs + sy[2] * sy[4] + sy[1] * sy[5] + 1) & ~1);
  for (int idx = tid; idx < 2 * n56; idx += MM6_THREADS) {
    const int side = idx >= n56, c = idx - side * n56;
    const int dg = c < sy[4] ? 4 : (c < sy[4] + sy[5] ? 5 : 6);
    const int col = dg == 4 ? c : (dg == 5 ? off5 + (c - sy[4]) : off6 + (c - sy[4] - sy[5]));
    float v = 0.0f;
    if (dg == 4 || (dg == 5 ? need5 : need6)) v = mom56[(item * 2 + side) * N56p + col];
    nq[idx] = v;
  }
  float* Gl = sm6 + ((2 * n56 + sy[3] * xs + sy[2] * sy[4] + sy[1] * sy[5] + 6 * MM6_WAVES + 2 + 3) & ~3);
  float* Bf4 = Gl + 128;
  float* X4 = Bf4 + sy[1] * sy[3];
  if (tid < 64) {
    const int i = tid >> 3, j = tid & 7;
    const double* pm = pairmat + ((size_t)b * P + (L + po)) * (d * d + 1);
    const float g = (i < d && j < d) ? (float)pm[i * d + j] : 0.0f;
    Gl[tid] = g;
    Gl[64 + j * 8 + i] = g;
  }
  double s2r = 0.0, s2c = 0.0;
  {
    const double* hr = whR + item * Mp;
    const double* hc = whC + item * Mp;
    const unsigned char* gf = gflag + item * (size_t)(Mp / MM_GROUP_ROWS);
    for (int m = tid; m < Mp; m += MM6_THREADS) {
      const double x = gf[m >> 6] ? hr[m] : 0.0, y = hc[m];
      s2r = fma(x, x, s2r); s2c = fma(y, y, s2c);
    }
  }
  __syncthreads();
  float G[64];
  auto load_G = [&](int transposed) __attribute__((always_inline)) {
#pragma unroll
    for (int q = 0; q < 16; ++q) {
      const float4 g4 = *reinterpret_cast<const float4*>(Gl + 64 * transposed + 4 * q);
      G[4 * q] = g4.x; G[4 * q + 1] = g4.y; G[4 * q + 2] = g4.z; G[4 * q + 3] = g4.w;
    }
  };
  const short* tabi = (const short*)tab;
  const float* mult2 = (const float*)(tab + (size_t)tb.n_i16 * 2) + tb.mult2;
  const float* mult3 = (const float*)(tab + (size_t)tb.n_i16 * 2) + tb.mult3;
  float acc5 = 0.0f, acc6 = 0.0f, dummy = 0.0f;
  if (need6) {
    const float* Q6 = nq + n56 + sy[4] + sy[5];
    const float* N6 = nq + sy[4] + sy[5];
    load_G(1);
    mm6_do<D8, 0, false, 0, NC, NW, 6, 0>(Q6, Bf, sy, tabi, tb, d, G, nullptr, 0, dummy, wave, lane);
    __syncthreads();
    mm6_do<D8, 1, false, 0, NC, NW, 5, 0>(Bf, A, sy, tabi, tb, d, G, nullptr, 0, dummy, wave, lane);
    __syncthreads();
    mm6_do<D8, 2, false, 1, NC, NW, 4, 121>(A, X, sy, tabi, tb, d, G, mult3, xs, dummy, wave, lane);
    __syncthreads();
    load_G(0);
    mm6_do<D8, 0, true, 0, NC, NW, 6, 0>(N6, Bf, sy, tabi, tb, d, G, nullptr, 0, dummy, wave, lane);
    __syncthreads();
    mm6_do<D8, 1, true, 0, NC, NW, 5, 0>(Bf, A, sy, tabi, tb, d, G, nullptr, 0, dummy, wave, lane);
    __syncthreads();
    mm6_do<D8, 2, true, 2, NC, NW, 4, 121>(A, X, sy, tabi, tb, d, G, nullptr, xs, acc6, wave, lane);
    __syncthreads();
  }
  float acc4 = 0.0f;
  {
    const float* Q5 = nq + n56 + sy[4];
    const float* N5 = nq + sy[4];
    const float* Q4 = nq + n56;
    const float* N4 = nq;
    const int xs4 = sy[2] + 1;
    load_G(1);
    if (need5) mm6_do<D8, 0, false, 0, NC, NW, 5, 0>(Q5, Bf, sy, tabi, tb, d, G, nullptr, 0, dummy, wave, lane);
    mm6_do<D8, 0, false, 0, NC, NW, 4, 0>(Q4, Bf4, sy, tabi, tb, d, G, nullptr, 0, dummy, wave, lane);
    __syncthreads();
    if (need5) mm6_do<D8, 1, false, 0, NC, NW, 4, 0>(Bf, A, sy, tabi, tb, d, G, nullptr, 0, dummy, wave, lane);
    mm6_do<D8, 1, false, 1, 1, NW, 3, 37>(Bf4, X4, sy, tabi, tb, d, G, mult2, xs4, dummy, wave, lane);
    __syncthreads();
    if (need5) {
      mm6_do<D8, 2, false, 1, 1, NW, 3, 121>(A, X, sy, tabi, tb, d, G, mult2, xs, dummy, wave, lane);
      __syncthreads();
    }
    load_G(0);
    if (need5) mm6_do<D8, 0, true, 0, NC, NW, 5, 0>(N5, Bf, sy, tabi, tb, d, G, nullptr, 0, dummy, wave, lane);
    mm6_do<D8, 0, true, 0, NC, NW, 4, 0>(N4, Bf4, sy, tabi, tb, d, G, nullptr, 0, dummy, wave, lane);
    __syncthreads();
    if (need5) mm6_do<D8, 1, true, 2, NC, NW, 4, 121>(Bf, X, sy, tabi, tb, d, G, nullptr, xs, acc5, wave, lane);
    mm6_do<D8, 1, true, 2, 1, NW, 3, 37>(Bf4, X4, sy, tabi, tb, d, G, nullptr, xs4, acc4, wave, lane);
  }
  double tot = (double)MM_C6_C1 * (double)acc4 + (double)MM_C6_C2 * (double)acc5 + (double)MM_C6_C3 * (double)acc6;
#pragma unroll
  for (int off = 32; off > 0; off >>= 1) {
    tot += __shfl_down(tot, off, 64); s2r += __shfl_down(s2r, off, 64); s2c += __shfl_down(s2c, off, 64);
  }
  double* redd = reinterpret_cast<double*>(red);
  if (lane == 0) { redd[wave * 3 + 0] = tot; redd[wave * 3 + 1] = s2r; redd[wave * 3 + 2] = s2c; }
  __syncthreads();
  if (tid == 0) {
    double t = 0.0, r2 = 0.0, c2 = 0.0;
    for (int w = 0; w < MM6_WAVES; ++w) { t += redd[w * 3]; r2 += redd[w * 3 + 1]; c2 += redd[w * 3 + 2]; }
    s56[item] = t;
    estS[item] = mm6_estS(bound2, need5, need6, r2, c2);
  }
  __syncthreads();
  }
}

template <bool D8>
__global__ __launch_bounds__(256) void k_spoly4(const float* __restrict__ mom56, int N56p, const double* __restrict__ pairmat,
                                                const double* __restrict__ zmax2, const unsigned int* __restrict__ amaxc,
                                                const unsigned char* __restrict__ gflag,
                                                const double* __restrict__ whR, const double* __restrict__ whC,
                                                const char* __restrict__ tab, MMTab56 tb, int L, int d_, int P, int Mp, int ntotal,
                                                const int* __restrict__ ilist,
                                                double* __restrict__ s56, float* __restrict__ estS) {
  extern __shared__ __align__(16) float sm4[];
  const int d = D8 ? 8 : d_;
  constexpr int NC0 = D8 ? 1 : MM6_NC;
  constexpr int NW = 4;
  const int tid = threadIdx.x;
  const int wave = __builtin_amdgcn_readfirstlane(tid >> 6), lane = tid & 63;
  const int Po = P - L;
  int sy[5];
#pragma unroll
  for (int k = 0; k < 5; ++k) sy[k] = mm_binom_i(d + k - 1, k);
  const int xs4 = sy[2] + 1;
  float* nq = sm4;
  float* Bf4 = nq + 2 * sy[4];
  float* X4 = Bf4 + sy[1] * sy[3];
  float* Gl = sm4 + ((2 * sy[4] + sy[1] * sy[3] + sy[2] * xs4 + 3) & ~3);
  double* redd = reinterpret_cast<double*>(Gl + 128);
  const short* tabi = (const short*)tab;
  const float* mult2 = (const float*)(tab + (size_t)tb.n_i16 * 2) + tb.mult2;
  const int nitems = __builtin_amdgcn_readfirstlane(ilist[2]);
  for (int li = blockIdx.x; li < nitems; li += gridDim.x) {
    const size_t item = (size_t)__builtin_amdgcn_readfirstlane(ilist[4 + ntotal - 1 - li]);
    const int b = (int)(item / Po), po = (int)(item - (size_t)b * Po);
    int a, a2;
    mm6_decode_pair_o(po, L, a, a2);
    const float bound2 = mm_collapse_bound2(amaxc[item], zmax2[a2]);
    for (int idx = tid; idx < 2 * sy[4]; idx += 256) {
      const int side = idx >= sy[4], c = idx - side * sy[4];
      nq[idx] = mom56[(item * 2 + side) * N56p + c];
    }
    if (tid < 64) {
      const int i = tid >> 3, j = tid & 7;
      const double* pm = pairmat + ((size_t)b * P + (L + po)) * (d * d + 1);
      const float g = (i < d && j < d) ? (float)pm[i * d + j] : 0.0f;
      Gl[tid] = g;
      Gl[64 + j * 8 + i] = g;
    }
    double s2r = 0.0, s2c = 0.0;
    {
      const double* hr = whR + item * Mp;
      const double* hc = whC + item * Mp;
      const unsigned char* gf = gflag + item * (size_t)(Mp / MM_GROUP_ROWS);
      for (int m = tid; m < Mp; m += 256) {
        const double x = gf[m >> 6] ? hr[m] : 0.0, y = hc[m];
        s2r = fma(x, x, s2r); s2c = fma(y, y, s2c);
      }
    }
    __syncthreads();
    float G[64];
    auto load_G = [&](int transposed) __attribute__((always_inline)) {
#pragma unroll
      for (int q = 0; q < 16; ++q) {
        const float4 g4 = *reinterpret_cast<const float4*>(Gl + 64 * transposed + 4 * q);
        G[4 * q] = g4.x; G[4 * q + 1] = g4.y; G[4 * q + 2] = g4.z; G[4 * q + 3] = g4.w;
      }
    };
    float acc4 = 0.0f, dummy = 0.0f;
    const float* Q4 = nq + sy[4];
    const float* N4 = nq;
    load_G(1);
    mm6_do<D8, 0, false, 0, NC0, NW, 4, 0>(Q4, Bf4, sy, tabi, tb, d, G, nullptr, 0, dummy, wave, lane);
    __syncthreads();
    mm6_do<D8, 1, false, 1, 1, NW, 3, 37>(Bf4, X4, sy, tabi, tb, d, G, mult2, xs4, dummy, wave, lane);
    __syncthreads();
    load_G(0);
    mm6_do<D8, 0, true, 0, NC0, NW, 4, 0>(N4, Bf4, sy, tabi, tb, d, G, nullptr, 0, dummy, wave, lane);
    __syncthreads();
    mm6_do<D8, 1, true, 2, 1, NW, 3, 37>(Bf4, X4, sy, tabi, tb, d, G, nullptr, xs4, acc4, wave, lane);
    double tot = (double)MM_C6_C1 * (double)acc4;
#pragma unroll
    for (int off = 32; off > 0; off >>= 1) {
      tot += __shfl_down(tot, off, 64); s2r += __shfl_down(s2r, off, 64); s2c += __shfl_down(s2c, off, 64);
    }
    if (lane == 0) { redd[wave * 3 + 0] = tot; redd[wave * 3 + 1] = s2r; redd[wave * 3 + 2] = s2c; }
    __syncthreads();
    if (tid == 0) {
      double t = 0.0, r2 = 0.0, c2 = 0.0;
      for (int w = 0; w < NW; ++w) { t += redd[w * 3]; r2 += redd[w * 3 + 1]; c2 += redd[w * 3 + 2]; }
      s56[item] = t;
      estS[item] = mm6_estS(bound2, false, false, r2, c2);
    }
    __syncthreads();
  }
}

int mm_launch_moments56(const char* packed, const MMModelLayout& ml, char* ws, const MMWorkspaceLayout& wl,
                        int B, int L, int d, int allow, int old_spoly56, hipStream_t stream) {
  const int N56p = mm_moment56_cols(d);
  if (N56p <= 0 || wl.Po <= 0) return 0;
  if (allow) {
    const int nrb = ((L - 1) * B + MM6_TB - 1) / MM6_TB, ncb = N56p / MM6_TB;
    const long long nwork_ll = (long long)L * ncb * nrb;
    if (nwork_ll <= 0 || nwork_ll > 0x7fffffffLL) return MM_E_DIM;
    if ((size_t)B * wl.Po * 4 * wl.Mp >= 0xffffffffull || (size_t)L * 2 * N56p * wl.Mp >= 0xffffffffull) return MM_E_DIM;
    const size_t shm = 2 * MM6_STAGE_BYTES + MM6_TB * sizeof(int);
    static std::atomic<unsigned long long> attr_done{0ull};
    int dev = 0;
    if (hipGetDevice(&dev) != hipSuccess) dev = 64;
    const unsigned long long bit = (dev >= 0 && dev < 64) ? (1ull << dev) : 0ull;
    if (!bit || !(attr_done.load() & bit)) {
      const hipError_t ea = hipFuncSetAttribute((const void*)k_wmom56_gemm, hipFuncAttributeMaxDynamicSharedMemorySize, (int)shm);
      if (ea != hipSuccess) return (int)ea;
      attr_done.fetch_or(bit);
    }
    hipLaunchKernelGGL(k_wmom56_gemm, dim3((int)nwork_ll), dim3(256), shm, stream, (const unsigned short*)(ws + wl.wsp),
                       (const unsigned short*)(packed + ml.Zm56), N56p, L, wl.Mp, B, wl.Po, nrb, ncb, (int)nwork_ll,
                       mm_moment56_off5(d) / MM6_TB, mm_moment56_off6(d) / MM6_TB,
                       (const int*)(ws + wl.gperm), (float*)(ws + wl.mom56));
    hipError_t e = hipGetLastError();
    if (e != hipSuccess) return (int)e;
  }
  const int nitem = B * wl.Po;
  int* ilist = (int*)(ws + wl.ilist);
  {
    const hipError_t em = hipMemsetAsync(ilist, 0, 16, stream);
    if (em != hipSuccess) return (int)em;
  }
  hipLaunchKernelGGL(k_item_classes, dim3((nitem + 255) / 256), dim3(256), 0, stream, (const unsigned int*)(ws + wl.amaxc),
                     (const double*)(packed + ml.zmax2), L, wl.Po, nitem, allow, ilist, (double*)(ws + wl.s56), (float*)(ws + wl.estS));
  {
    const hipError_t ec = hipGetLastError();
    if (ec != hipSuccess) return (int)ec;
  }
  if (!allow) return 0;
  int sy[7];
  for (int k = 0; k < 7; ++k) sy[k] = mm_mono_count(k, d);
  size_t nfl = (size_t)2 * (sy[4] + sy[5] + sy[6]) + (size_t)sy[3] * (sy[3] + 1) + (size_t)sy[2] * sy[4] + (size_t)sy[1] * sy[5] + 6 * MM6_WAVES + 128 + 16
               + (size_t)sy[1] * sy[3] + (size_t)sy[2] * (sy[2] + 1);
  nfl = (nfl + 1) & ~(size_t)1;
  const size_t shm = nfl * sizeof(float);
  static std::atomic<unsigned long long> attr2_done{0ull};
  static std::atomic<int> ncu_cached[64];
  int dev = 0;
  if (hipGetDevice(&dev) != hipSuccess) dev = 64;
  const unsigned long long bit2 = (dev >= 0 && dev < 64) ? (1ull << dev) : 0ull;
  int ncu = bit2 ? ncu_cached[dev].load() : 0;
  if (!bit2 || !(attr2_done.load() & bit2)) {
    hipError_t ea = hipFuncSetAttribute((const void*)k_spoly56<false>, hipFuncAttributeMaxDynamicSharedMemorySize, 160 * 1024);
    if (ea == hipSuccess) ea = hipFuncSetAttribute((const void*)k_spoly56<true>, hipFuncAttributeMaxDynamicSharedMemorySize, 160 * 1024);
    if (ea != hipSuccess) return (int)ea;
    int v = 0;
    if (hipDeviceGetAttribute(&v, hipDeviceAttributeMultiprocessorCount, dev < 64 ? dev : 0) != hipSuccess || v <= 0) v = 256;
    ncu = v;
    if (bit2) { ncu_cached[dev].store(v); attr2_done.fetch_or(bit2); }
  }
  if (ncu <= 0) ncu = 256;
  const int g56 = nitem < ncu ? nitem : ncu, g4 = nitem < 8 * ncu ? nitem : 8 * ncu;
  const bool d8 = d == 8 && !old_spoly56;
  hipLaunchKernelGGL((d8 ? k_spoly56<true> : k_spoly56<false>), dim3(g56), dim3(MM6_THREADS), shm, stream, (const float*)(ws + wl.mom56), N56p,
                     (const double*)(ws + wl.pairmat), (const double*)(packed + ml.zmax2), (const unsigned int*)(ws + wl.amaxc),
                     (const unsigned char*)(ws + wl.gflag), (const double*)(ws + wl.whR), (const double*)(ws + wl.whC),
                     packed + ml.tab56, mm_tab56(d), L, d, wl.P, wl.Mp, (const int*)ilist, (double*)(ws + wl.s56), (float*)(ws + wl.estS));
  {
    const hipError_t e5 = hipGetLastError();
    if (e5 != hipSuccess) return (int)e5;
  }
  const size_t shm4 = (size_t)(((2 * sy[4] + sy[1] * sy[3] + sy[2] * (sy[2] + 1) + 3) & ~3) + 128 + 2 * 3 * 4 + 8) * sizeof(float);
  hipLaunchKernelGGL((d8 ? k_spoly4<true> : k_spoly4<false>), dim3(g4), dim3(256), shm4, stream, (const float*)(ws + wl.mom56), N56p,
                     (const double*)(ws + wl.pairmat), (const double*)(packed + ml.zmax2), (const unsigned int*)(ws + wl.amaxc),
                     (const unsigned char*)(ws + wl.gflag), (const double*)(ws + wl.whR), (const double*)(ws + wl.whC),
                     packed + ml.tab56, mm_tab56(d), L, d, wl.P, wl.Mp, nitem, (const int*)ilist, (double*)(ws + wl.s56),
                     (float*)(ws + wl.estS));
  hipError_t e = hipGetLastError();
  return e == hipSuccess ? 0 : (int)e;
}
```

Before: 47030 rollout step-elements/s (B*H per rollout second).

## Prefetch spoly stage index tables and moments into registers ahead of barriers

```diff
diff --git a/__graft_entry__.py b/__graft_entry__.py
--- a/__graft_entry__.py
+++ b/__graft_entry__.py
@@ -17,6 +17,7 @@
   subprocess.run(["bash", os.path.join(ROOT, "tests", "hostcheck", "build_predict.sh")], check=True)
   subprocess.run(["bash", os.path.join(ROOT, "tests", "hostcheck", "build_gram_stats.sh")], check=True)
   subprocess.run(["bash", os.path.join(ROOT, "tests", "hostcheck", "build_lanes.sh")], check=True)
+  subprocess.run(["bash", os.path.join(ROOT, "tests", "hostcheck", "build_ws_layout.sh")], check=True)
   subprocess.run(["bash", os.path.join(ROOT, "tests", "devcheck", "build.sh")], check=True)
   import gpflowpilco_amd
   from gpflowpilco_amd import _lib
diff --git a/gpflowpilco_amd/_lib.py b/gpflowpilco_amd/_lib.py
--- a/gpflowpilco_amd/_lib.py
+++ b/gpflowpilco_amd/_lib.py
@@ -23,6 +23,7 @@
 MM_ISTAGE_OLD_SKIP_BOUND = 1 << 26
 MM_ISTAGE_NO_BOUND_SKIP = 1 << 27
 MM_ISTAGE_OLD_WMOM = 1 << 28
+MM_ISTAGE_OLD_SPOLY_LOADS = 1 << 29
 
 ERRORS = {
     -1: "MM_E_ARG: NULL pointer or non-positive size",
diff --git a/gpflowpilco_amd/csrc/mm_common.h b/gpflowpilco_amd/csrc/mm_common.h
--- a/gpflowpilco_amd/csrc/mm_common.h
+++ b/gpflowpilco_amd/csrc/mm_common.h
@@ -16,6 +16,7 @@
 #define MM_ISTAGE_OLD_SKIP_BOUND (1 << 26)
 #define MM_ISTAGE_NO_BOUND_SKIP (1 << 27)
 #define MM_ISTAGE_OLD_WMOM (1 << 28)
+#define MM_ISTAGE_OLD_SPOLY_LOADS (1 << 29)
 
 #define MM_PW_KERNELS 3
 
diff --git a/gpflowpilco_amd/csrc/mm_moments.hip b/gpflowpilco_amd/csrc/mm_moments.hip
--- a/gpflowpilco_amd/csrc/mm_moments.hip
+++ b/gpflowpilco_amd/csrc/mm_moments.hip
@@ -442,6 +442,7 @@
 }
 static inline int mm_spw_slice(int ncs) { return 512 + 16 + 64 + 2 + 2 * ncs + 64 + 8; }
 
+template <bool PRE>
 __global__ __launch_bounds__(64 * MM_SPW_WAVES) void k_spoly_wave8(const double* __restrict__ mom, int KMp, const double* __restrict__ pairmat,
                                                                    const double* __restrict__ zbar, const unsigned int* __restrict__ amax,
                                                                    const unsigned int* __restrict__ amaxc, const float* __restrict__ mu,
@@ -466,19 +467,52 @@
   double* qh = nh + ncs;
   double* Gs = qh + ncs;
   double* dmu = Gs + DK * DK;
-  const bool coll = allow_collapse && mm_item_collapsed(amaxc[(size_t)b * Po + po]);
-  const int nmax = coll ? DEG : 2;
-  {
+  const double* nm = mom + (((size_t)b * Po + po) * 2 + 0) * MM_MOM_SPLIT * KMp;
+  const double* qm = mom + (((size_t)b * Po + po) * 2 + 1) * MM_MOM_SPLIT * KMp;
+  const double* pm = pairmat + ((size_t)b * P + p) * (d * d + 1);
+  bool coll;
+  if constexpr (PRE) {
+    const int gi = lane >> LB, gj = lane & (DK - 1);
+    const bool gok = gi < d && gj < d, mok = lane < DK && lane < d;
+    const unsigned int wc = amaxc[(size_t)b * Po + po], wa = amax[(size_t)b * Po + po];
+    const double g = pm[gok ? gi * d + gj : 0];
+    const float mu_l = mu[(size_t)b * d + (mok ? lane : 0)];
+    const double zb_l = zbar[a * d + (mok ? lane : 0)];
+    coll = allow_collapse && mm_item_collapsed(wc);
     const int ncol = coll ? off4 : off3;
-    const double* nm = mom + (((size_t)b * Po + po) * 2 + 0) * MM_MOM_SPLIT * KMp;
-    const double* qm = mom + (((size_t)b * Po + po) * 2 + 1) * MM_MOM_SPLIT * KMp;
+    constexpr int NK = 3;
+    double vn[NK][MM_MOM_SPLIT], vq[NK][MM_MOM_SPLIT];
+#pragma unroll
+    for (int i = 0; i < NK; ++i) {
+      const int k = lane + 64 * i, kc = k < ncol ? k : 0;
+#pragma unroll
+      for (int t = 0; t < MM_MOM_SPLIT; ++t) { vn[i][t] = nm[t * KMp + kc]; vq[i][t] = qm[t * KMp + kc]; }
+    }
+    Gs[lane] = gok ? g : 0.0;
+    if (lane < DK) dmu[lane] = (mok && !mm_rows_recentred(wa)) ? (double)mu_l - zb_l : 0.0;
+#pragma unroll
+    for (int i = 0; i < NK; ++i) {
+      const int k = lane + 64 * i;
+      double sn = 0.0, sq = 0.0;
+#pragma unroll
+      for (int t = 0; t < MM_MOM_SPLIT; ++t) { sn += vn[i][t]; sq += vq[i][t]; }
+      if (k < ncol) { nh[k] = sn; qh[k] = sq; }
+    }
+    for (int k = lane + 64 * NK; k < ncol; k += 64) {
+      double sn = 0.0, sq = 0.0;
+#pragma unroll
+      for (int t = 0; t < MM_MOM_SPLIT; ++t) { sn += nm[t * KMp + k]; sq += qm[t * KMp + k]; }
+      nh[k] = sn; qh[k] = sq;
+    }
+  } else {
+    coll = allow_collapse && mm_item_collapsed(amaxc[(size_t)b * Po + po]);
+    const int ncol = coll ? off4 : off3;
     for (int k = lane; k < ncol; k += 64) {
       double sn = 0.0, sq = 0.0;
 #pragma unroll
       for (int t = 0; t < MM_MOM_SPLIT; ++t) { sn += nm[t * KMp + k]; sq += qm[t * KMp + k]; }
       nh[k] = sn; qh[k] = sq;
     }
-    const double* pm = pairmat + ((size_t)b * P + p) * (d * d + 1);
     {
       const int i = lane >> LB, j = lane & (DK - 1);
       Gs[lane] = (i < d && j < d) ? pm[i * d + j] : 0.0;
@@ -486,6 +520,7 @@
     const bool rcen = mm_rows_recentred(amax[(size_t)b * Po + po]);
     if (lane < DK) dmu[lane] = (lane < d && !rcen) ? (double)mu[(size_t)b * d + lane] - zbar[a * d + lane] : 0.0;
   }
+  const int nmax = coll ? DEG : 2;
   mm_wave_sync_m();
   double Gr[64];
 #pragma unroll
@@ -608,7 +643,7 @@
 }
 
 int mm_launch_moments56(const char* packed, const MMModelLayout& ml, char* ws, const MMWorkspaceLayout& wl,
-                        int B, int L, int d, int allow, int old_spoly56, hipStream_t stream);
+                        int B, int L, int d, int allow, int old_spoly56, int old_loads, hipStream_t stream);
 
 int mm_launch_moments(const char* packed, const MMModelLayout& ml, char* ws, const MMWorkspaceLayout& wl,
                       int B, int L, int d, const void* mu_f32, int flags, hipStream_t stream) {
@@ -660,7 +695,8 @@
     const int ncs = (off4 + 7) & ~7;
     const int slice = mm_spw_slice(ncs);
     const int nitem = B * wl.Po;
-    hipLaunchKernelGGL(k_spoly_wave8, dim3((nitem + MM_SPW_WAVES - 1) / MM_SPW_WAVES), dim3(64 * MM_SPW_WAVES),
+    const auto kw8 = (flags & MM_ISTAGE_OLD_SPOLY_LOADS) ? k_spoly_wave8<false> : k_spoly_wave8<true>;
+    hipLaunchKernelGGL(kw8, dim3((nitem + MM_SPW_WAVES - 1) / MM_SPW_WAVES), dim3(64 * MM_SPW_WAVES),
                        (size_t)MM_SPW_WAVES * slice * sizeof(double), stream, (const double*)mom, ml.KMp,
                        (const double*)(ws + wl.pairmat), (const double*)(packed + ml.zbar), (const unsigned int*)(ws + wl.amax),
                        (const unsigned int*)(ws + wl.amaxc), (const float*)mu_f32, L, d, wl.P, B, allow, off1, off2, off3, off4,
@@ -676,7 +712,8 @@
     const hipError_t es = hipMemsetAsync(ws + wl.estS, 0, (size_t)B * wl.Po * sizeof(float), stream);
     return es == hipSuccess ? 0 : (int)es;
   }
-  return mm_launch_moments56(packed, ml, ws, wl, B, L, d, some ? 1 : 0, (flags & MM_ISTAGE_OLD_SPOLY56) ? 1 : 0, stream);
+  return mm_launch_moments56(packed, ml, ws, wl, B, L, d, some ? 1 : 0, (flags & MM_ISTAGE_OLD_SPOLY56) ? 1 : 0,
+                             (flags & MM_ISTAGE_OLD_SPOLY_LOADS) ? 1 : 0, stream);
 }
 
 __global__ void k_offdiag_stats(const unsigned int* __restrict__ amax, const double* __restrict__ zmax2,
diff --git a/gpflowpilco_amd/csrc/mm_moments6.hip b/gpflowpilco_amd/csrc/mm_moments6.hip
--- a/gpflowpilco_amd/csrc/mm_moments6.hip
+++ b/gpflowpilco_amd/csrc/mm_moments6.hip
@@ -210,10 +210,50 @@
 #ifndef MM6_NC
 #define MM6_NC 2
 #endif
-template <int K, bool TRANSG, int MODE, int NC = MM6_NC, int NW = MM6_WAVES>
+typedef unsigned int mm6_u4 __attribute__((ext_vector_type(4), aligned(8)));
+template <int NC> struct mm6_pre { mm6_u4 w[NC]; float mj[NC]; };
+
+template <int MODE, int NC>
+__device__ __forceinline__ void mm6_pre_arrived(mm6_pre<NC>& pre) {
+#pragma unroll
+  for (int q = 0; q < NC; ++q) {
+    asm volatile("" : "+v"(pre.w[q]));
+    if constexpr (MODE == 1) asm volatile("" : "+v"(pre.mj[q]));
+  }
+}
+
+template <int NC>
+__device__ __forceinline__ void mm6_pre_offsets(const mm6_pre<NC>& pre, int (&off)[NC][8], float (&mj)[NC]) {
+#pragma unroll
+  for (int q = 0; q < NC; ++q) {
+#pragma unroll
+    for (int j = 0; j < 4; ++j) {
+      off[q][2 * j] = (int)(short)(pre.w[q][j] & 0xffffu);
+      off[q][2 * j + 1] = (int)pre.w[q][j] >> 16;
+    }
+    mj[q] = pre.mj[q];
+  }
+}
+
+template <int K, int MODE, int NC>
+__device__ __forceinline__ void mm6_request(mm6_pre<NC>& pre, int nI, int nJp, const short* __restrict__ ins,
+                                            const float* __restrict__ multJ, int wave, int lane) {
+  int c = K == 0 ? wave : (int)(((float)wave + 0.5f) * (1.0f / (float)nI));
+  c = __builtin_amdgcn_readfirstlane(c);
+#pragma unroll
+  for (int q = 0; q < NC; ++q) {
+    const int Jp = (c * NC + q) * 64 + lane;
+    const int Jc = Jp < nJp ? Jp : nJp - 1;
+    pre.w[q] = *reinterpret_cast<const mm6_u4*>(ins + (size_t)Jc * 8);
+    pre.mj[q] = 0.0f;
+    if constexpr (MODE == 1) pre.mj[q] = multJ[Jc];
+  }
+}
+
+template <int K, bool TRANSG, int MODE, int NC = MM6_NC, int NW = MM6_WAVES, bool PRE = false>
 __device__ __forceinline__ void mm6_step(const float* __restrict__ Tin, int nJin, int nI, float* __restrict__ Tout, int nJp,
                                          const short* __restrict__ ins, int d, const float (&G)[64], const float* __restrict__ multJ,
-                                         int xs, float& acc, int wave, int lane) {
+                                         int xs, float& acc, int wave, int lane, const mm6_pre<NC>& pre) {
   const int chunks = (nJp + 64 * NC - 1) / (64 * NC);
   auto dots = [&](auto i0c, const float (&v)[NC][8], float (&s)[NC][8]) __attribute__((always_inline)) {
     constexpr int I0 = decltype(i0c)::value;
@@ -265,6 +305,17 @@
   float mj[NC];
 #pragma unroll
   for (int q = 0; q < NC; ++q) { Jc[q] = 0; jv[q] = false; mj[q] = 0.0f; }
+  if constexpr (PRE) {
+    cprev = K == 0 ? wave : (int)(((float)wave + 0.5f) * rnI);
+    cprev = __builtin_amdgcn_readfirstlane(cprev);
+#pragma unroll
+    for (int q = 0; q < NC; ++q) {
+      const int Jp = (cprev * NC + q) * 64 + lane;
+      jv[q] = Jp < nJp;
+      Jc[q] = jv[q] ? Jp : nJp - 1;
+    }
+    mm6_pre_offsets<NC>(pre, off, mj);
+  }
   for (int u = wave; u < nunit; u += NW) {
     int c = K == 0 ? u : (int)(((float)u + 0.5f) * rnI);
     c = __builtin_amdgcn_readfirstlane(c);
@@ -302,9 +353,35 @@
 }
 constexpr int mm6_sym8(int k) { return mm6_cbinom(8 + k - 1, k); }
 
-template <int K, int MODE, int NJIN, int NJP, int XS, int NC, int NW>
+template <int K, int MODE, int NJP, int NC, int NW>
+__device__ __forceinline__ int mm6_first_c8(int wave) {
+  constexpr int NI = mm6_sym8(K);
+  constexpr int CH = (NJP + 64 * NC - 1) / (64 * NC);
+  if constexpr (CH == 1) return 0;
+  else if constexpr (NI == 1) return wave;
+  else if constexpr (MODE != 2 && NW % CH == 0) return wave % CH;
+  else return wave / NI;
+}
+
+template <int K, int MODE, int NJP, int NC, int NW>
+__device__ __forceinline__ void mm6_request8(mm6_pre<NC>& pre, const short* __restrict__ ins, const float* __restrict__ multJ,
+                                             int wave, int lane) {
+  asm volatile("" : "+v"(lane));
+  const int c = mm6_first_c8<K, MODE, NJP, NC, NW>(wave);
+#pragma unroll
+  for (int q = 0; q < NC; ++q) {
+    const int Jp = (c * NC + q) * 64 + lane;
+    const int Jc = Jp < NJP ? Jp : NJP - 1;
+    pre.w[q] = *reinterpret_cast<const mm6_u4*>(ins + (size_t)Jc * 8);
+    pre.mj[q] = 0.0f;
+    if constexpr (MODE == 1) pre.mj[q] = multJ[Jc];
+  }
+}
+
+template <int K, int MODE, int NJIN, int NJP, int XS, int NC, int NW, bool PRE = false>
 __device__ __forceinline__ void mm6_step8(const float* __restrict__ Tin_, float* __restrict__ Tout_, const short* __restrict__ ins,
-                                          const float (&G)[64], const float* __restrict__ multJ, float& acc, int wave, int lane) {
+                                          const float (&G)[64], const float* __restrict__ multJ, float& acc, int wave, int lane,
+                                          const mm6_pre<NC>& pre) {
   asm volatile("" : "+v"(lane));
   unsigned a_in = (unsigned)(size_t)(const mm6_lds_f*)Tin_, a_out = (unsigned)(size_t)(mm6_lds_f*)Tout_;
   asm volatile("" : "+s"(a_in));
@@ -334,6 +411,24 @@
       if constexpr (MODE == 1) mj[q] = multJ[Jc[q]];
     }
   };
+  auto take_c = [&](int c) __attribute__((always_inline)) {
+    if constexpr (PRE) {
+#pragma unroll
+      for (int q = 0; q < NC; ++q) {
+        const int Jp = (c * NC + q) * 64 + lane;
+        jv[q] = Jp < NJP;
+        Jc[q] = jv[q] ? Jp : NJP - 1;
+      }
+      mm6_pre_offsets<NC>(pre, off, mj);
+#pragma unroll
+      for (int q = 0; q < NC; ++q) {
+#pragma unroll
+        for (int j = 0; j < 8; ++j) asm volatile("" : "+v"(off[q][j]));
+      }
+    } else {
+      load_c(c);
+    }
+  };
   auto body = [&](auto i0c, int I, bool first) __attribute__((always_inline)) {
     constexpr int I0 = decltype(i0c)::value;
     const mm6_lds_f* tin = Tin + I * NJIN;
@@ -423,22 +518,23 @@
   };
   if constexpr (CH == 1) {
     if (wave < NI) {
-      load_c(0);
+      take_c(0);
       for (int I = wave; I < NI; I += NW)
         if (jv[0]) unit(I);
     }
   } else if constexpr (NI == 1) {
     for (int c = wave; c < CH; c += NW) {
-      load_c(c);
+      if (PRE && c == wave) take_c(c); else load_c(c);
       if (jv[0]) unit(0);
     }
   } else if constexpr (MODE != 2 && NW % CH == 0) {
     const int c = wave % CH;
-    load_c(c);
+    take_c(c);
     for (int I = wave / CH; I < NI; I += NW / CH)
       if (jv[0]) unit(I);
   } else {
     int cprev = -1;
+    if constexpr (PRE) { cprev = wave / NI; take_c(cprev); }
     for (int u = wave; u < CH * NI; u += NW) {
       const int c = u / NI, I = u - c * NI;
       if (c != cprev) { cprev = c; load_c(c); }
@@ -447,15 +543,48 @@
   }
 }
 
-template <bool D8, int K, bool TRANSG, int MODE, int NC, int NW, int KIN, int XS8>
+template <bool D8, int K, bool TRANSG, int MODE, int NC, int NW, int KIN, int XS8, bool PRE = false>
 __device__ __forceinline__ void mm6_do(const float* __restrict__ Tin, float* __restrict__ Tout, const int* sy, const short* __restrict__ tabi,
                                        const MMTab56& tb, int d, const float (&G)[64], const float* __restrict__ multJ, int xs,
-                                       float& acc, int wave, int lane) {
+                                       float& acc, int wave, int lane, const mm6_pre<NC>& pre = mm6_pre<NC>{}) {
   if constexpr (D8)
-    mm6_step8<K, MODE, mm6_sym8(KIN), mm6_sym8(KIN - 1), XS8, NC, NW>(Tin, Tout, tabi + tb.ins[KIN - 1], G, multJ, acc, wave, lane);
+    mm6_step8<K, MODE, mm6_sym8(KIN), mm6_sym8(KIN - 1), XS8, NC, NW, PRE>(Tin, Tout, tabi + tb.ins[KIN - 1], G, multJ, acc, wave, lane, pre);
   else
-    mm6_step<K, TRANSG, MODE, NC, NW>(Tin, sy[KIN], sy[K], Tout, sy[KIN - 1], tabi + tb.ins[KIN - 1], d, G, multJ, xs, acc, wave, lane);
-}
+    mm6_step<K, TRANSG, MODE, NC, NW, PRE>(Tin, sy[KIN], sy[K], Tout, sy[KIN - 1], tabi + tb.ins[KIN - 1], d, G, multJ, xs, acc, wave, lane, pre);
+}
+
+template <bool D8, int K, int MODE, int NC, int NW, int KIN>
+__device__ __forceinline__ void mm6_req(mm6_pre<NC>& pre, const int* sy, const short* __restrict__ tabi, const MMTab56& tb,
+                                        const float* __restrict__ multJ, int wave, int lane) {
+  if constexpr (D8) mm6_request8<K, MODE, mm6_sym8(KIN - 1), NC, NW>(pre, tabi + tb.ins[KIN - 1], multJ, wave, lane);
+  else mm6_request<K, MODE, NC>(pre, sy[K], sy[KIN - 1], tabi + tb.ins[KIN - 1], multJ, wave, lane);
+}
+
+template <int W> struct mm6_vecw { typedef float type __attribute__((ext_vector_type(W))); };
+constexpr int mm6_vec_width(int n) { return n <= 4 ? 4 : (n <= 8 ? 8 : 16); }
+
+template <int T, int U>
+struct mm6_s2_batch {
+  unsigned char f[U];
+  double x[U], y[U];
+  __device__ __forceinline__ void issue(const unsigned char* __restrict__ gf, const double* __restrict__ hr, const double* __restrict__ hc,
+                                        int m0, int Mp) {
+#pragma unroll
+    for (int u = 0; u < U; ++u) {
+      const int m = m0 + u * T, mc = m < Mp ? m : 0;
+      f[u] = gf[mc >> 6]; x[u] = hr[mc]; y[u] = hc[mc];
+    }
+  }
+  __device__ __forceinline__ void add(int m0, int Mp, double& s2r, double& s2c) const {
+#pragma unroll
+    for (int u = 0; u < U; ++u) {
+      const bool in = m0 + u * T < Mp;
+      const double xx = f[u] ? x[u] : 0.0;
+      const double r = fma(xx, xx, s2r), c = fma(y[u], y[u], s2c);
+      s2r = in ? r : s2r; s2c = in ? c : s2c;
+    }
+  }
+};
 
 __global__ __launch_bounds__(256) void k_item_classes(const unsigned int* __restrict__ amaxc, const double* __restrict__ zmax2,
                                                       int L, int Po, int n, int allow, int* __restrict__ ilist,
@@ -490,7 +619,7 @@
   return (float)fmin((double)MM_C6_SYS2 * (amp * amp) * r2 * c2, 3.0e38);
 }
 
-template <bool D8>
+template <bool D8, bool PRE>
 __global__ __launch_bounds__(MM6_THREADS) void k_spoly56(const float* __restrict__ mom56, int N56p, const double* __restrict__ pairmat,
                                                  const double* __restrict__ zmax2, const unsigned int* __restrict__ amaxc,
                                                  const unsigned char* __restrict__ gflag,
@@ -524,35 +653,86 @@
   float* A = X + sy[3] * xs;
   float* Bf = A + sy[2] * sy[4];
   float* red = sm6 + ((2 * n56 + sy[3] * xs + sy[2] * sy[4] + sy[1] * sy[5] + 1) & ~1);
-  for (int idx = tid; idx < 2 * n56; idx += MM6_THREADS) {
-    const int side = idx >= n56, c = idx - side * n56;
+  const short* tabi = (const short*)tab;
+  const float* mult2 = (const float*)(tab + (size_t)tb.n_i16 * 2) + tb.mult2;
+  const float* mult3 = (const float*)(tab + (size_t)tb.n_i16 * 2) + tb.mult3;
+  auto nq_col = [&](int idx, int& side, int& col) __attribute__((always_inline)) {
+    side = idx >= n56;
+    const int c = idx - side * n56;
     const int dg = c < sy[4] ? 4 : (c < sy[4] + sy[5] ? 5 : 6);
-    const int col = dg == 4 ? c : (dg == 5 ? off5 + (c - sy[4]) : off6 + (c - sy[4] - sy[5]));
-    float v = 0.0f;
-    if (dg == 4 || (dg == 5 ? need5 : need6)) v = mom56[(item * 2 + side) * N56p + col];
-    nq[idx] = v;
-  }
+    col = dg == 4 ? c : (dg == 5 ? off5 + (c - sy[4]) : off6 + (c - sy[4] - sy[5]));
+    return dg == 4 || (dg == 5 ? need5 : need6);
+  };
   float* Gl = sm6 + ((2 * n56 + sy[3] * xs + sy[2] * sy[4] + sy[1] * sy[5] + 6 * MM6_WAVES + 2 + 3) & ~3);
   float* Bf4 = Gl + 128;
   float* X4 = Bf4 + sy[1] * sy[3];
-  if (tid < 64) {
-    const int i = tid >> 3, j = tid & 7;
-    const double* pm = pairmat + ((size_t)b * P + (L + po)) * (d * d + 1);
-    const float g = (i < d && j < d) ? (float)pm[i * d + j] : 0.0f;
-    Gl[tid] = g;
-    Gl[64 + j * 8 + i] = g;
-  }
+  const double* pm = pairmat + ((size_t)b * P + (L + po)) * (d * d + 1);
+  const double* hr = whR + item * Mp;
+  const double* hc = whC + item * Mp;
+  const unsigned char* gf = gflag + item * (size_t)(Mp / MM_GROUP_ROWS);
   double s2r = 0.0, s2c = 0.0;
-  {
-    const double* hr = whR + item * Mp;
-    const double* hc = whC + item * Mp;
-    const unsigned char* gf = gflag + item * (size_t)(Mp / MM_GROUP_ROWS);
+  mm6_pre<NC> p0 = {};
+  mm6_pre<1> p1 = {};
+  if constexpr (PRE) {
+    int tid = threadIdx.x;
+    asm volatile("" : "+v"(tid));
+    constexpr int S2U = 4;
+    mm6_s2_batch<MM6_THREADS, S2U> sb;
+    sb.issue(gf, hr, hc, tid, Mp);
+    const int gi = tid >> 3, gj = tid & 7;
+    const bool gok = tid < 64 && gi < d && gj < d;
+    const double gd = pm[gok ? gi * d + gj : 0];
+    constexpr int NQL = (2 * (mm6_sym8(4) + mm6_sym8(5) + mm6_sym8(6)) + MM6_THREADS - 1) / MM6_THREADS;
+    static_assert(NQL <= 16, "the moments of one thread as one register tuple");
+    typename mm6_vecw<mm6_vec_width(NQL)>::type r = 0.0f;
+    const float* mrow = mom56 + item * 2 * N56p;
+#pragma unroll
+    for (int q = 0; q < NQL; ++q) {
+      const int idx = tid + q * MM6_THREADS;
+      int side, col;
+      const bool ld = nq_col(idx, side, col) && idx < 2 * n56;
+      r[q] = mrow[ld ? side * N56p + col : 0];
+    }
+    if (need6) mm6_req<D8, 0, 0, NC, NW, 6>(p0, sy, tabi, tb, nullptr, wave, lane);
+    else mm6_req<D8, 0, 0, NC, NW, 5>(p0, sy, tabi, tb, nullptr, wave, lane);
+    asm volatile("" : "+v"(r));
+#pragma unroll
+    for (int q = 0; q < NQL; ++q) {
+      const int idx = tid + q * MM6_THREADS;
+      int side, col;
+      const bool ld = nq_col(idx, side, col);
+      if (idx < 2 * n56) nq[idx] = ld ? r[q] : 0.0f;
+    }
+    if (tid < 64) {
+      const float g = gok ? (float)gd : 0.0f;
+      Gl[tid] = g;
+      Gl[64 + gj * 8 + gi] = g;
+    }
+    sb.add(tid, Mp, s2r, s2c);
+    for (int m0 = tid + S2U * MM6_THREADS; m0 < Mp; m0 += S2U * MM6_THREADS) {
+      sb.issue(gf, hr, hc, m0, Mp);
+      sb.add(m0, Mp, s2r, s2c);
+    }
+  } else {
+    for (int idx = tid; idx < 2 * n56; idx += MM6_THREADS) {
+      int side, col;
+      float v = 0.0f;
+      if (nq_col(idx, side, col)) v = mom56[(item * 2 + side) * N56p + col];
+      nq[idx] = v;
+    }
+    if (tid < 64) {
+      const int i = tid >> 3, j = tid & 7;
+      const float g = (i < d && j < d) ? (float)pm[i * d + j] : 0.0f;
+      Gl[tid] = g;
+      Gl[64 + j * 8 + i] = g;
+    }
     for (int m = tid; m < Mp; m += MM6_THREADS) {
       const double x = gf[m >> 6] ? hr[m] : 0.0, y = hc[m];
       s2r = fma(x, x, s2r); s2c = fma(y, y, s2c);
     }
   }
   __syncthreads();
+  if constexpr (PRE) mm6_pre_arrived<0>(p0);
   float G[64];
   auto load_G = [&](int transposed) __attribute__((always_inline)) {
 #pragma unroll
@@ -561,27 +741,36 @@
       G[4 * q] = g4.x; G[4 * q + 1] = g4.y; G[4 * q + 2] = g4.z; G[4 * q + 3] = g4.w;
     }
   };
-  const short* tabi = (const short*)tab;
-  const float* mult2 = (const float*)(tab + (size_t)tb.n_i16 * 2) + tb.mult2;
-  const float* mult3 = (const float*)(tab + (size_t)tb.n_i16 * 2) + tb.mult3;
   float acc5 = 0.0f, acc6 = 0.0f, dummy = 0.0f;
   if (need6) {
     const float* Q6 = nq + n56 + sy[4] + sy[5];
     const float* N6 = nq + sy[4] + sy[5];
     load_G(1);
-    mm6_do<D8, 0, false, 0, NC, NW, 6, 0>(Q6, Bf, sy, tabi, tb, d, G, nullptr, 0, dummy, wave, lane);
-    __syncthreads();
-    mm6_do<D8, 1, false, 0, NC, NW, 5, 0>(Bf, A, sy, tabi, tb, d, G, nullptr, 0, dummy, wave, lane);
-    __syncthreads();
-    mm6_do<D8, 2, false, 1, NC, NW, 4, 121>(A, X, sy, tabi, tb, d, G, mult3, xs, dummy, wave, lane);
-    __syncthreads();
+    mm6_do<D8, 0, false, 0, NC, NW, 6, 0, PRE>(Q6, Bf, sy, tabi, tb, d, G, nullptr, 0, dummy, wave, lane, p0);
+    if constexpr (PRE) mm6_req<D8, 1, 0, NC, NW, 5>(p0, sy, tabi, tb, nullptr, wave, lane);
+    __syncthreads();
+    if constexpr (PRE) mm6_pre_arrived<0>(p0);
+    mm6_do<D8, 1, false, 0, NC, NW, 5, 0, PRE>(Bf, A, sy, tabi, tb, d, G, nullptr, 0, dummy, wave, lane, p0);
+    if constexpr (PRE) mm6_req<D8, 2, 1, NC, NW, 4>(p0, sy, tabi, tb, mult3, wave, lane);
+    __syncthreads();
+    if constexpr (PRE) mm6_pre_arrived<1>(p0);
+    mm6_do<D8, 2, false, 1, NC, NW, 4, 121, PRE>(A, X, sy, tabi, tb, d, G, mult3, xs, dummy, wave, lane, p0);
+    if constexpr (PRE) mm6_req<D8, 0, 0, NC, NW, 6>(p0, sy, tabi, tb, nullptr, wave, lane);
+    __syncthreads();
+    if constexpr (PRE) mm6_pre_arrived<0>(p0);
     load_G(0);
-    mm6_do<D8, 0, true, 0, NC, NW, 6, 0>(N6, Bf, sy, tabi, tb, d, G, nullptr, 0, dummy, wave, lane);
-    __syncthreads();
-    mm6_do<D8, 1, true, 0, NC, NW, 5, 0>(Bf, A, sy, tabi, tb, d, G, nullptr, 0, dummy, wave, lane);
-    __syncthreads();
-    mm6_do<D8, 2, true, 2, NC, NW, 4, 121>(A, X, sy, tabi, tb, d, G, nullptr, xs, acc6, wave, lane);
-    __syncthreads();
+    mm6_do<D8, 0, true, 0, NC, NW, 6, 0, PRE>(N6, Bf, sy, tabi, tb, d, G, nullptr, 0, dummy, wave, lane, p0);
+    if constexpr (PRE) mm6_req<D8, 1, 0, NC, NW, 5>(p0, sy, tabi, tb, nullptr, wave, lane);
+    __syncthreads();
+    if constexpr (PRE) mm6_pre_arrived<0>(p0);
+    mm6_do<D8, 1, true, 0, NC, NW, 5, 0, PRE>(Bf, A, sy, tabi, tb, d, G, nullptr, 0, dummy, wave, lane, p0);
+    if constexpr (PRE) mm6_req<D8, 2, 2, NC, NW, 4>(p0, sy, tabi, tb, nullptr, wave, lane);
+    __syncthreads();
+    if constexpr (PRE) mm6_pre_arrived<2>(p0);
+    mm6_do<D8, 2, true, 2, NC, NW, 4, 121, PRE>(A, X, sy, tabi, tb, d, G, nullptr, xs, acc6, wave, lane, p0);
+    if constexpr (PRE) mm6_req<D8, 0, 0, NC, NW, 5>(p0, sy, tabi, tb, nullptr, wave, lane);
+    __syncthreads();
+    if constexpr (PRE) mm6_pre_arrived<0>(p0);
   }
   float acc4 = 0.0f;
   {
@@ -591,21 +780,29 @@
     const float* N4 = nq;
     const int xs4 = sy[2] + 1;
     load_G(1);
-    if (need5) mm6_do<D8, 0, false, 0, NC, NW, 5, 0>(Q5, Bf, sy, tabi, tb, d, G, nullptr, 0, dummy, wave, lane);
+    if (need5) mm6_do<D8, 0, false, 0, NC, NW, 5, 0, PRE>(Q5, Bf, sy, tabi, tb, d, G, nullptr, 0, dummy, wave, lane, p0);
     mm6_do<D8, 0, false, 0, NC, NW, 4, 0>(Q4, Bf4, sy, tabi, tb, d, G, nullptr, 0, dummy, wave, lane);
-    __syncthreads();
-    if (need5) mm6_do<D8, 1, false, 0, NC, NW, 4, 0>(Bf, A, sy, tabi, tb, d, G, nullptr, 0, dummy, wave, lane);
+    if constexpr (PRE) { if (need5) mm6_req<D8, 1, 0, NC, NW, 4>(p0, sy, tabi, tb, nullptr, wave, lane); }
+    __syncthreads();
+    if constexpr (PRE) mm6_pre_arrived<0>(p0);
+    if (need5) mm6_do<D8, 1, false, 0, NC, NW, 4, 0, PRE>(Bf, A, sy, tabi, tb, d, G, nullptr, 0, dummy, wave, lane, p0);
     mm6_do<D8, 1, false, 1, 1, NW, 3, 37>(Bf4, X4, sy, tabi, tb, d, G, mult2, xs4, dummy, wave, lane);
-    __syncthreads();
+    if constexpr (PRE) { if (need5) mm6_req<D8, 2, 1, 1, NW, 3>(p1, sy, tabi, tb, mult2, wave, lane); }
+    __syncthreads();
+    if constexpr (PRE) mm6_pre_arrived<1>(p1);
     if (need5) {
-      mm6_do<D8, 2, false, 1, 1, NW, 3, 121>(A, X, sy, tabi, tb, d, G, mult2, xs, dummy, wave, lane);
+      mm6_do<D8, 2, false, 1, 1, NW, 3, 121, PRE>(A, X, sy, tabi, tb, d, G, mult2, xs, dummy, wave, lane, p1);
+      if constexpr (PRE) mm6_req<D8, 0, 0, NC, NW, 5>(p0, sy, tabi, tb, nullptr, wave, lane);
       __syncthreads();
+      if constexpr (PRE) mm6_pre_arrived<0>(p0);
     }
     load_G(0);
-    if (need5) mm6_do<D8, 0, true, 0, NC, NW, 5, 0>(N5, Bf, sy, tabi, tb, d, G, nullptr, 0, dummy, wave, lane);
+    if (need5) mm6_do<D8, 0, true, 0, NC, NW, 5, 0, PRE>(N5, Bf, sy, tabi, tb, d, G, nullptr, 0, dummy, wave, lane, p0);
     mm6_do<D8, 0, true, 0, NC, NW, 4, 0>(N4, Bf4, sy, tabi, tb, d, G, nullptr, 0, dummy, wave, lane);
-    __syncthreads();
-    if (need5) mm6_do<D8, 1, true, 2, NC, NW, 4, 121>(Bf, X, sy, tabi, tb, d, G, nullptr, xs, acc5, wave, lane);
+    if constexpr (PRE) { if (need5) mm6_req<D8, 1, 2, NC, NW, 4>(p0, sy, tabi, tb, nullptr, wave, lane); }
+    __syncthreads();
+    if constexpr (PRE) mm6_pre_arrived<2>(p0);
+    if (need5) mm6_do<D8, 1, true, 2, NC, NW, 4, 121, PRE>(Bf, X, sy, tabi, tb, d, G, nullptr, xs, acc5, wave, lane, p0);
     mm6_do<D8, 1, true, 2, 1, NW, 3, 37>(Bf4, X4, sy, tabi, tb, d, G, nullptr, xs4, acc4, wave, lane);
   }
   double tot = (double)MM_C6_C1 * (double)acc4 + (double)MM_C6_C2 * (double)acc5 + (double)MM_C6_C3 * (double)acc6;
@@ -626,7 +823,7 @@
   }
 }
 
-template <bool D8>
+template <bool D8, bool PRE>
 __global__ __launch_bounds__(256) void k_spoly4(const float* __restrict__ mom56, int N56p, const double* __restrict__ pairmat,
                                                 const double* __restrict__ zmax2, const unsigned int* __restrict__ amaxc,
                                                 const unsigned char* __restrict__ gflag,
@@ -659,28 +856,67 @@
     int a, a2;
     mm6_decode_pair_o(po, L, a, a2);
     const float bound2 = mm_collapse_bound2(amaxc[item], zmax2[a2]);
-    for (int idx = tid; idx < 2 * sy[4]; idx += 256) {
-      const int side = idx >= sy[4], c = idx - side * sy[4];
-      nq[idx] = mom56[(item * 2 + side) * N56p + c];
-    }
-    if (tid < 64) {
-      const int i = tid >> 3, j = tid & 7;
-      const double* pm = pairmat + ((size_t)b * P + (L + po)) * (d * d + 1);
-      const float g = (i < d && j < d) ? (float)pm[i * d + j] : 0.0f;
-      Gl[tid] = g;
-      Gl[64 + j * 8 + i] = g;
-    }
+    const double* pm = pairmat + ((size_t)b * P + (L + po)) * (d * d + 1);
+    const double* hr = whR + item * Mp;
+    const double* hc = whC + item * Mp;
+    const unsigned char* gf = gflag + item * (size_t)(Mp / MM_GROUP_ROWS);
     double s2r = 0.0, s2c = 0.0;
-    {
-      const double* hr = whR + item * Mp;
-      const double* hc = whC + item * Mp;
-      const unsigned char* gf = gflag + item * (size_t)(Mp / MM_GROUP_ROWS);
+    mm6_pre<NC0> p0 = {};
+    mm6_pre<1> p1 = {};
+    if constexpr (PRE) {
+      int tid = threadIdx.x;
+      asm volatile("" : "+v"(tid));
+      constexpr int S2U = 4;
+      mm6_s2_batch<256, S2U> sb;
+      sb.issue(gf, hr, hc, tid, Mp);
+      const int gi = tid >> 3, gj = tid & 7;
+      const bool gok = tid < 64 && gi < d && gj < d;
+      const double gd = pm[gok ? gi * d + gj : 0];
+      constexpr int NQL = (2 * mm6_sym8(4) + 255) / 256;
+      static_assert(NQL <= 16, "the moments of one thread as one register tuple");
+      typename mm6_vecw<mm6_vec_width(NQL)>::type r = 0.0f;
+      const float* mrow = mom56 + item * 2 * N56p;
+#pragma unroll
+      for (int q = 0; q < NQL; ++q) {
+        const int idx = tid + q * 256;
+        const int side = idx >= sy[4], c = idx - side * sy[4];
+        r[q] = mrow[idx < 2 * sy[4] ? side * N56p + c : 0];
+      }
+      mm6_req<D8, 0, 0, NC0, NW, 4>(p0, sy, tabi, tb, nullptr, wave, lane);
+      asm volatile("" : "+v"(r));
+#pragma unroll
+      for (int q = 0; q < NQL; ++q) {
+        const int idx = tid + q * 256;
+        if (idx < 2 * sy[4]) nq[idx] = r[q];
+      }
+      if (tid < 64) {
+        const float g = gok ? (float)gd : 0.0f;
+        Gl[tid] = g;
+        Gl[64 + gj * 8 + gi] = g;
+      }
+      sb.add(tid, Mp, s2r, s2c);
+      for (int m0 = tid + S2U * 256; m0 < Mp; m0 += S2U * 256) {
+        sb.issue(gf, hr, hc, m0, Mp);
+        sb.add(m0, Mp, s2r, s2c);
+      }
+    } else {
+      for (int idx = tid; idx < 2 * sy[4]; idx += 256) {
+        const int side = idx >= sy[4], c = idx - side * sy[4];
+        nq[idx] = mom56[(item * 2 + side) * N56p + c];
+      }
+      if (tid < 64) {
+        const int i = tid >> 3, j = tid & 7;
+        const float g = (i < d && j < d) ? (float)pm[i * d + j] : 0.0f;
+        Gl[tid] = g;
+        Gl[64 + j * 8 + i] = g;
+      }
       for (int m = tid; m < Mp; m += 256) {
         const double x = gf[m >> 6] ? hr[m] : 0.0, y = hc[m];
         s2r = fma(x, x, s2r); s2c = fma(y, y, s2c);
       }
     }
     __syncthreads();
+    if constexpr (PRE) mm6_pre_arrived<0>(p0);
     float G[64];
     auto load_G = [&](int transposed) __attribute__((always_inline)) {
 #pragma unroll
@@ -693,14 +929,20 @@
     const float* Q4 = nq + sy[4];
     const float* N4 = nq;
     load_G(1);
-    mm6_do<D8, 0, false, 0, NC0, NW, 4, 0>(Q4, Bf4, sy, tabi, tb, d, G, nullptr, 0, dummy, wave, lane);
-    __syncthreads();
-    mm6_do<D8, 1, false, 1, 1, NW, 3, 37>(Bf4, X4, sy, tabi, tb, d, G, mult2, xs4, dummy, wave, lane);
-    __syncthreads();
+    mm6_do<D8, 0, false, 0, NC0, NW, 4, 0, PRE>(Q4, Bf4, sy, tabi, tb, d, G, nullptr, 0, dummy, wave, lane, p0);
+    if constexpr (PRE) mm6_req<D8, 1, 1, 1, NW, 3>(p1, sy, tabi, tb, mult2, wave, lane);
+    __syncthreads();
+    if constexpr (PRE) mm6_pre_arrived<1>(p1);
+    mm6_do<D8, 1, false, 1, 1, NW, 3, 37, PRE>(Bf4, X4, sy, tabi, tb, d, G, mult2, xs4, dummy, wave, lane, p1);
+    if constexpr (PRE) mm6_req<D8, 0, 0, NC0, NW, 4>(p0, sy, tabi, tb, nullptr, wave, lane);
+    __syncthreads();
+    if constexpr (PRE) mm6_pre_arrived<0>(p0);
     load_G(0);
-    mm6_do<D8, 0, true, 0, NC0, NW, 4, 0>(N4, Bf4, sy, tabi, tb, d, G, nullptr, 0, dummy, wave, lane);
-    __syncthreads();
-    mm6_do<D8, 1, true, 2, 1, NW, 3, 37>(Bf4, X4, sy, tabi, tb, d, G, nullptr, xs4, acc4, wave, lane);
+    mm6_do<D8, 0, true, 0, NC0, NW, 4, 0, PRE>(N4, Bf4, sy, tabi, tb, d, G, nullptr, 0, dummy, wave, lane, p0);
+    if constexpr (PRE) mm6_req<D8, 1, 2, 1, NW, 3>(p1, sy, tabi, tb, nullptr, wave, lane);
+    __syncthreads();
+    if constexpr (PRE) mm6_pre_arrived<2>(p1);
+    mm6_do<D8, 1, true, 2, 1, NW, 3, 37, PRE>(Bf4, X4, sy, tabi, tb, d, G, nullptr, xs4, acc4, wave, lane, p1);
     double tot = (double)MM_C6_C1 * (double)acc4;
 #pragma unroll
     for (int off = 32; off > 0; off >>= 1) {
@@ -719,7 +961,7 @@
 }
 
 int mm_launch_moments56(const char* packed, const MMModelLayout& ml, char* ws, const MMWorkspaceLayout& wl,
-                        int B, int L, int d, int allow, int old_spoly56, hipStream_t stream) {
+                        int B, int L, int d, int allow, int old_spoly56, int old_loads, hipStream_t stream) {
   const int N56p = mm_moment56_cols(d);
   if (N56p <= 0 || wl.Po <= 0) return 0;
   if (allow) {
@@ -770,8 +1012,10 @@
   const unsigned long long bit2 = (dev >= 0 && dev < 64) ? (1ull << dev) : 0ull;
   int ncu = bit2 ? ncu_cached[dev].load() : 0;
   if (!bit2 || !(attr2_done.load() & bit2)) {
-    hipError_t ea = hipFuncSetAttribute((const void*)k_spoly56<false>, hipFuncAttributeMaxDynamicSharedMemorySize, 160 * 1024);
-    if (ea == hipSuccess) ea = hipFuncSetAttribute((const void*)k_spoly56<true>, hipFuncAttributeMaxDynamicSharedMemorySize, 160 * 1024);
+    hipError_t ea = hipSuccess;
+    for (const void* fn : {(const void*)k_spoly56<false, false>, (const void*)k_spoly56<true, false>, (const void*)k_spoly56<false, true>,
+                           (const void*)k_spoly56<true, true>})
+      if (ea == hipSuccess) ea = hipFuncSetAttribute(fn, hipFuncAttributeMaxDynamicSharedMemorySize, 160 * 1024);
     if (ea != hipSuccess) return (int)ea;
     int v = 0;
     if (hipDeviceGetAttribute(&v, hipDeviceAttributeMultiprocessorCount, dev < 64 ? dev : 0) != hipSuccess || v <= 0) v = 256;
@@ -781,7 +1025,10 @@
   if (ncu <= 0) ncu = 256;
   const int g56 = nitem < ncu ? nitem : ncu, g4 = nitem < 8 * ncu ? nitem : 8 * ncu;
   const bool d8 = d == 8 && !old_spoly56;
-  hipLaunchKernelGGL((d8 ? k_spoly56<true> : k_spoly56<false>), dim3(g56), dim3(MM6_THREADS), shm, stream, (const float*)(ws + wl.mom56), N56p,
+  const bool pre = !old_loads;
+  const auto k56 = d8 ? (pre ? k_spoly56<true, true> : k_spoly56<true, false>) : (pre ? k_spoly56<false, true> : k_spoly56<false, false>);
+  const auto k4 = d8 ? (pre ? k_spoly4<true, true> : k_spoly4<true, false>) : (pre ? k_spoly4<false, true> : k_spoly4<false, false>);
+  hipLaunchKernelGGL(k56, dim3(g56), dim3(MM6_THREADS), shm, stream, (const float*)(ws + wl.mom56), N56p,
                      (const double*)(ws + wl.pairmat), (const double*)(packed + ml.zmax2), (const unsigned int*)(ws + wl.amaxc),
                      (const unsigned char*)(ws + wl.gflag), (const double*)(ws + wl.whR), (const double*)(ws + wl.whC),
                      packed + ml.tab56, mm_tab56(d), L, d, wl.P, wl.Mp, (const int*)ilist, (double*)(ws + wl.s56), (float*)(ws + wl.estS));
@@ -790,7 +1037,7 @@
     if (e5 != hipSuccess) return (int)e5;
   }
   const size_t shm4 = (size_t)(((2 * sy[4] + sy[1] * sy[3] + sy[2] * (sy[2] + 1) + 3) & ~3) + 128 + 2 * 3 * 4 + 8) * sizeof(float);
-  hipLaunchKernelGGL((d8 ? k_spoly4<true> : k_spoly4<false>), dim3(g4), dim3(256), shm4, stream, (const float*)(ws + wl.mom56), N56p,
+  hipLaunchKernelGGL(k4, dim3(g4), dim3(256), shm4, stream, (const float*)(ws + wl.mom56), N56p,
                      (const double*)(ws + wl.pairmat), (const double*)(packed + ml.zmax2), (const unsigned int*)(ws + wl.amaxc),
                      (const unsigned char*)(ws + wl.gflag), (const double*)(ws + wl.whR), (const double*)(ws + wl.whC),
                      packed + ml.tab56, mm_tab56(d), L, d, wl.P, wl.Mp, nitem, (const int*)ilist, (double*)(ws + wl.s56),
```

Result: no change. 47650 rollout step-elements/s (B*H per rollout second), median of 6 (+1.3%).
